# Bebra777228/PolGen-RVC

Measured on AMD Instinct MI355X. Metric: real-time-factor (audio-sec/wall-sec) per GPU, 30s@16kHz RMVPE->48kHz, higher is better.
Workload: dtype f32 (conv products as 3 fp16 MFMAs of a hi/lo split, fp32 accumulate; fp32 elsewhere)

## Files before the change

### include/rvcx.h

```cpp
#ifndef RVCX_H
#define RVCX_H
#include <stdint.h>

#ifdef __cplusplus
extern "C" {
#endif

typedef struct rvcx_ctx rvcx_ctx;

typedef struct {
  const char* name;
  const void* data;
  int32_t dtype;
  int32_t ndim;
  int64_t shape[4];
} rvcx_tensor;

typedef struct {
  int32_t inter_channels, hidden_channels, filter_channels, n_heads, n_layers, kernel_size;
  int32_t n_resblocks;
  int32_t res_kernels[4];
  int32_t res_dilations[4][3];
  int32_t n_ups;
  int32_t up_rates[6], up_kernels[6];
// ... 175 lines not shown
  float reverb_rm_size, reverb_wet, reverb_dry, reverb_damping, reverb_width;
  float low_shelf_gain, high_shelf_gain;
  float compressor_ratio, compressor_threshold;
  float noise_gate_threshold, noise_gate_ratio, noise_gate_attack, noise_gate_release;
  float chorus_rate_hz, chorus_depth, chorus_centre_delay_ms, chorus_feedback, chorus_mix;
  int32_t sample_rate, channels;
} rvcx_fx_params;
int rvcx_fx_chain(rvcx_ctx*, int B, const float* const* x_hd, const int64_t* n, const rvcx_fx_params*, float* const* y_hd);
int rvcx_op_fx_highpass(rvcx_ctx*, const float* x_hd, int64_t n, int channels, int sr, float fc, float* y_hd);
int rvcx_op_fx_compressor(rvcx_ctx*, const float* x_hd, int64_t n, int channels, int sr, float ratio, float threshold_db,
                          float attack_ms, float release_ms, float* y_hd, float* env_hd);
int rvcx_op_fx_gate(rvcx_ctx*, const float* x_hd, int64_t n, int channels, int sr, float threshold_db, float ratio,
                    float attack_ms, float release_ms, float* y_hd, float* env_hd);
int rvcx_op_fx_reverb(rvcx_ctx*, const float* x_hd, int64_t n, int channels, int sr, float room_size, float damping, float wet,
                      float dry, float width, float* y_hd);
int rvcx_op_fx_shelf(rvcx_ctx*, const float* x_hd, int64_t n, int channels, int sr, int high, float gain_db, float fc, float Q,
                     float* y_hd);
int rvcx_op_fx_chorus(rvcx_ctx*, const float* x_hd, int64_t n, int channels, int sr, float rate_hz, float depth,
                      float centre_delay_ms, float feedback, float mix, float* y_hd);
int rvcx_op_fx_mix(rvcx_ctx*, const int16_t* vocal_hd, int64_t n_v, const int16_t* inst_hd, int64_t n_i, float vocal_gain_db,
                   float inst_gain_db, int16_t* out_hd);
int rvcx_fx_chunk(void);
int rvcx_fx_last_passes(rvcx_ctx*, int32_t* passes3);
float rvcx_fx_cte(double ms, int sr);
int rvcx_fx_delay(int sr, int D);
int rvcx_fx_coeffs(int kind, int sr, double fc, double Q, double gain_db, float* coef5);
int rvcx_fx_highpass_host(const float* x, int64_t n, int sr, float fc, float* y);
int rvcx_fx_biquad_host(const float* x, int64_t n, const float* coef5, float* y);
int rvcx_fx_follower_host(const float* x, int64_t n, int square, int sqrt_out, float c_attack, float c_release, float* env);
int rvcx_fx_compressor_host(const float* x, int64_t n, int sr, float ratio, float threshold_db, float attack_ms,
                            float release_ms, float* y, float* env);
int rvcx_fx_gate_host(const float* x, int64_t n, int sr, float threshold_db, float ratio, float attack_ms, float release_ms,
                      float* y, float* env);
int rvcx_fx_comb_host(const float* in, int64_t n, int D, float fb, float d, float* out);
int rvcx_fx_allpass_host(const float* in, int64_t n, int D, float* out);
int rvcx_fx_chorus_host(const float* x, int64_t n, int sr, float rate_hz, float depth, float centre_delay_ms, float feedback,
                        float mix, float* y);
int rvcx_fx_mix_host(const int16_t* vocal, int64_t n_v, const int16_t* inst, int64_t n_i, float vocal_gain_db,
                     float inst_gain_db, int16_t* out);

int rvcx_stream_open_fx(rvcx_ctx*, int model_id, const rvcx_stream_cfg*, const rvcx_stream_io*, const rvcx_fx_params* fx,
                        const rvcx_params* p, const int32_t* sid, const float* pitch, int* stream_id);
int rvcx_stream_out_channels(rvcx_ctx*, int stream_id);
int rvcx_stream_set_fx(rvcx_ctx*, int stream_id, const rvcx_fx_params*);
int rvcx_stream_last_fx_ms(rvcx_ctx*, int stream_id, float* ms8);
int rvcx_op_stream_fx(rvcx_ctx*, const float* x_hd, int S, int64_t frames, int channels, int sr, int block_frames,
                      const rvcx_fx_params* fx, uint32_t stage_mask, float* y_hd);
int rvcx_fx_reverb_host(const float* x, int64_t n, int sr, float room_size, float damping, float wet, float dry, float width,
                        float* y);

int rvcx_last_timing(rvcx_ctx*, float* ms9);
int rvcx_conv_profile(rvcx_ctx*, int begin, int64_t* launches, double* flops, double* ms, int32_t* bm,
                      int32_t* bn, int32_t* kind, int cap);
const char* rvcx_conv_profile_csv(rvcx_ctx*);
int rvcx_device_info(int device, char* name, int name_cap, int64_t* total_bytes);
int rvcx_mem_info(rvcx_ctx*, int64_t* free_bytes, int64_t* total_bytes);
int64_t rvcx_fp32_reruns(rvcx_ctx*);
int64_t rvcx_fp32_layers(rvcx_ctx*);
int rvcx_fp32_pinned(rvcx_ctx*, char* buf, int cap);
int64_t rvcx_gru_fallbacks(rvcx_ctx*);
int rvcx_gru_publish_probe(rvcx_ctx*);
int64_t rvcx_index_exhaustive(rvcx_ctx*);

int rvcx_kmeans(rvcx_ctx*, const float* x_hd, int64_t n, int dim, const float* init_hd, int k, int iters,
                float* centroids_hd, int32_t* assign_hd, int32_t* counts_hd, double* objective, int32_t* splits);
int rvcx_ivf_assign(rvcx_ctx*, const float* x_hd, int64_t n, int dim, const float* centroids_hd, int nlist,
                    int32_t* assign_hd);
int rvcx_index_features(rvcx_ctx*, int B, const float* wav_hd, int64_t n, int out_dim, float* feats_hd);
int64_t rvcx_kmeans_exhaustive(rvcx_ctx*);

int rvcx_debug_inject(rvcx_ctx*, int what);
double rvcx_flop_counter(rvcx_ctx*, int reset);
void* rvcx_stream(rvcx_ctx*);

int rvcx_op_fcpe_post(rvcx_ctx*, const float* raw_hd, int F_in, int p_len, double pitch, double f0_min, double f0_max,
                      int32_t* coarse, float* f0);
int rvcx_op_conv1d(rvcx_ctx*, const float* x, const float* w, const float* bias, const float* res,
                   float* y, int B, int Cin, int Tin, int Cout, int K, int stride, int dil,
                   int pad_left, int Tout, int groups, int pre_lrelu, float pre_slope, int act,
                   float act_slope, const int32_t* lens_in, const int32_t* lens_out);
int rvcx_op_resblock_pair(rvcx_ctx*, const float* x, const float* w1, const float* b1, const float* w2,
                          const float* b2, float* y, int B, int C, int T, int K, int dil, float slope, int fused,
                          const int32_t* lens);
int rvcx_op_resblock3(rvcx_ctx*, const float* x, const float* w1, const float* b1, const float* w2, const float* b2,
                      float* y, int B, int C, int T, const int32_t* dils, float slope, const int32_t* lens);
int rvcx_bench_resblock_pair(rvcx_ctx*, int B, int C, int T, int K, int dil, int fused, int iters,
                             float* ms_per_launch);
int rvcx_bench_conv1d(rvcx_ctx*, int B, int Cin, int Tin, int Cout, int K, int stride, int dil, int groups,
                      int iters, float* ms_per_launch);
int rvcx_conv_override(int tile, int variant, int splitk);
int rvcx_op_convtranspose1d(rvcx_ctx*, const float* x, const float* w, const float* bias, float* y,
                            int B, int Cin, int Tin, int Cout, int K, int stride, int pad,
                            int pre_lrelu, float pre_slope);
int rvcx_op_conv2d3x3(rvcx_ctx*, const float* x, const float* w, const float* bias, const float* res,
                      float* y, int B, int Cin, int H, int W, int Cout, int act);
int rvcx_op_convblock2d(rvcx_ctx*, const float* x, const float* w1, const float* b1, const float* w2, const float* b2,
                        const float* wsc, const float* bsc, float* y, int B, int Cin, int Cout, int H, int W,
                        const int32_t* rows);
int rvcx_op_convtranspose2d(rvcx_ctx*, const float* x, const float* w, const float* bias, float* y,
                            int B, int Cin, int H, int W, int Cout, int act);
int rvcx_op_attention(rvcx_ctx*, const float* q, const float* k, const float* v, float* out, int B,
                      int H, int D, int T, float scale, const float* emb_rel_k,
                      const float* emb_rel_v, int window, const int32_t* lens);
int rvcx_op_gemm_tm(rvcx_ctx*, const float* x_cf, const float* w, const float* bias, const float* res_tm, int B, int T,
                    int Cin, int Cout, int act, int exact_fp32, float* y_tm, float* y_cf, float* y_split);
int rvcx_bench_gemm(rvcx_ctx*, int64_t rows, int Cin, int Cout, int iters, float* ms_per_launch);
int rvcx_op_layernorm_tm(rvcx_ctx*, const float* x, const float* gamma, const float* beta, float* y, float* y_split,
                         int64_t rows, int C, float eps);
int rvcx_op_layernorm_c(rvcx_ctx*, const float* x, const float* gamma, const float* beta, float* y,
                        int B, int C, int T, float eps);
int rvcx_op_groupnorm_gelu(rvcx_ctx*, const float* x, const float* gamma, const float* beta, int B, int C, int T, float eps,
                           const int32_t* lens, float* y, float* stats, float* y_split);
int rvcx_op_hubert_conv0(rvcx_ctx*, const float* wav, const float* w, const float* gamma, const float* beta, int B, int C,
                         int n, int K, int stride, float eps, const int32_t* lens, int fused, float* stats, float* y_split,
                         uint16_t* raw_split);
int rvcx_op_sine_source(rvcx_ctx*, const float* f0, const float* noise, const float* lin_wb, int B, int T, int upp, float sr,
                        const int32_t* lens, float* har);
int rvcx_op_randn(rvcx_ctx*, int64_t n, uint64_t seed, uint64_t offset, float* out);
int rvcx_op_reflect_pad(rvcx_ctx*, const float* x, int B, int n, int p, const int32_t* ns, float* y);
int rvcx_op_mel_post(rvcx_ctx*, const float* mel, int B, int nmel, int F, int Tp, const float* bn, const int32_t* fs,
                     const int32_t* tps, float* out);
int rvcx_op_decode_f0(rvcx_ctx*, const float* sal, int B, int T, int ld, float thred, float f0_min, float f0_max, float* f0);
int rvcx_op_avgpool2(rvcx_ctx*, const float* x, int planes, int H, int Wp, int64_t x_ps, int64_t y_ps, float* y);
int rvcx_op_gru_input(rvcx_ctx*, const float* x, int B, int C, int T, int Wp, float* y);
int rvcx_op_upsample_protect(rvcx_ctx*, const float* feats, const float* feats0, const float* pitchf, int C, int Th, int p_len,
                             float protect, int use_protect, int ld_in, int ld_out, float* out);
int rvcx_op_bigru(rvcx_ctx*, const float* x, const float* w_ih, const float* w_hh, const float* b_ih,
                  const float* b_hh, const float* w_ih_r, const float* w_hh_r, const float* b_ih_r,
                  const float* b_hh_r, float* y, int B, int T, int I, int H);
int rvcx_op_highpass(rvcx_ctx*, const double* x, double* y, int64_t n);
int rvcx_highpass_exact(const double* x, double* y, int64_t n);

int64_t rvcx_flac_encode_bound(int64_t frames, int channels);
int64_t rvcx_flac_encode_s16(const int16_t* pcm, int64_t frames, int channels, int sample_rate, uint8_t* out, int64_t cap);
int rvcx_flac_info(const uint8_t* data, int64_t n, int64_t* frames, int32_t* channels, int32_t* sample_rate, int32_t* bits);
int64_t rvcx_flac_decode_s32(const uint8_t* data, int64_t n, int32_t* out, int64_t cap_samples);
const char* rvcx_flac_last_error(void);

#ifdef __cplusplus
}
#endif
#endif
```

### polgen-rvc_amd/_lib.py

```python
from __future__ import annotations

import ctypes as C
import os
import threading
import types
from typing import Optional, Sequence

import numpy as np

_HERE = os.path.dirname(os.path.abspath(__file__))
LIB_PATH = os.environ.get("RVCX_LIBRARY") or os.path.join(_HERE, "librvcx.so")


class RvcxError(RuntimeError):
    pass


class Tensor(C.Structure):
    _fields_ = [("name", C.c_char_p), ("data", C.c_void_p), ("dtype", C.c_int32),
                ("ndim", C.c_int32), ("shape", C.c_int64 * 4)]


class SynthCfg(C.Structure):
    _fields_ = [("inter_channels", C.c_int32), ("hidden_channels", C.c_int32),
# ... 49 lines not shown
class FxParams(C.Structure):
    _fields_ = [(k, C.c_float) for k in FX_FIELDS] + [("sample_rate", C.c_int32), ("channels", C.c_int32)]

    @classmethod
    def make(cls, values, sample_rate, channels=2):
        p = cls()
        if isinstance(values, dict):
            values = [values[k] for k in FX_FIELDS]
        if len(values) != len(FX_FIELDS):
            raise RvcxError(f"FxParams: {len(FX_FIELDS)} effect values expected, got {len(values)}")
        for k, v in zip(FX_FIELDS, values):
            setattr(p, k, float(v))
        p.sample_rate, p.channels = int(sample_rate), int(channels)
        return p


FX_UI_DEFAULTS = dict(reverb_rm_size=0.1, reverb_wet=0.1, reverb_dry=0.8, reverb_damping=0.9, reverb_width=1.0,
                      low_shelf_gain=0, high_shelf_gain=0, compressor_ratio=4, compressor_threshold=-12,
                      noise_gate_threshold=-40, noise_gate_ratio=8, noise_gate_attack=10, noise_gate_release=100,
                      chorus_rate_hz=0, chorus_depth=0, chorus_centre_delay_ms=0, chorus_feedback=0, chorus_mix=0)


class StreamIO(C.Structure):
    _fields_ = [("in_rate", C.c_int32), ("in_channels", C.c_int32), ("out_rate", C.c_int32), ("reserved", C.c_int32)]


def stream_resample_delay(sr_in: int, sr_out: int) -> int:
    return int(lib().rvcx_stream_resample_delay(int(sr_in), int(sr_out)))


class StreamCfg(C.Structure):
    _fields_ = [("n_streams", C.c_int32), ("block_frames", C.c_int32), ("context_frames", C.c_int32),
                ("crossfade_frames", C.c_int32), ("search_frames", C.c_int32)]


def head_from_rate(T: int, rate) -> int:
    return int(int(T) * (1.0 - float(np.float32(rate))))


def sola_reference(y, b, Lb, Lx, Ls, offset=None):
    y, b = np.asarray(y, np.float64), np.asarray(b, np.float64)
    Lb, Lx, Ls = int(Lb), int(Lx), int(Ls)
    assert y.shape == (Lb + Lx + Ls,) and b.shape == (Lx,)
    win = np.lib.stride_tricks.sliding_window_view(y[:Ls + Lx], Lx)
    den = np.sqrt((win * win).sum(1) + 1e-8)
    scores = (win @ b) / den
    mags = (np.abs(win) @ np.abs(b)) / den
    d = int(np.argmax(scores)) if offset is None else int(offset)
    out = y[d:d + Lb].copy()
    k = min(Lx, Lb)
    fin = np.sin(0.5 * np.pi * np.arange(Lx) / max(Lx - 1, 1)) ** 2
    out[:k] = y[d:d + k] * fin[:k] + b[:k] * (1.0 - fin[:k])
    return out, y[d + Lb:d + Lb + Lx].copy(), d, scores, mags


_lib = None

SYMBOLS = [
    "rvcx_create", "rvcx_destroy", "rvcx_last_error", "rvcx_version", "rvcx_load_hubert",
    "rvcx_load_rmvpe", "rvcx_index_exhaustive", "rvcx_load_crepe", "rvcx_crepe_frames", "rvcx_crepe_predict", "rvcx_op_crepe_decode", "rvcx_get_f0_crepe_x", "rvcx_load_fcpe", "rvcx_fcpe_f0", "rvcx_fcpe_frames", "rvcx_get_f0_fcpe_x", "rvcx_op_fcpe_post", "rvcx_load_synth", "rvcx_unload_synth", "rvcx_load_index", "rvcx_load_index_ivf",
    "rvcx_weights_regions", "rvcx_weights_adopt", "rvcx_weights_clone", "rvcx_rmvpe_f0", "rvcx_rmvpe_frames", "rvcx_rmvpe_mel", "rvcx_synth_infer_taps", "rvcx_hubert_features",
    "rvcx_hubert_frames", "rvcx_synth_infer", "rvcx_synth_infer_window", "rvcx_synth_dec_rf", "rvcx_synth_upp", "rvcx_index_blend",
    "rvcx_out_len", "rvcx_convert_batch", "rvcx_convert_batch_f64", "rvcx_micro_batch", "rvcx_bucket_length", "rvcx_last_micro_batches", "rvcx_last_cuts", "rvcx_noise_len",
    "rvcx_get_f0", "rvcx_get_f0_x", "rvcx_vc", "rvcx_vc_frames", "rvcx_last_timing",
    "rvcx_flop_counter", "rvcx_fp32_reruns", "rvcx_mem_info", "rvcx_conv_profile", "rvcx_conv_profile_csv", "rvcx_stream", "rvcx_op_conv1d", "rvcx_op_resblock_pair", "rvcx_bench_resblock_pair", "rvcx_bench_conv1d", "rvcx_conv_override", "rvcx_op_convtranspose1d",
    "rvcx_op_conv2d3x3", "rvcx_op_convblock2d", "rvcx_op_convtranspose2d", "rvcx_op_attention", "rvcx_op_layernorm_c",
    "rvcx_op_bigru", "rvcx_op_highpass", "rvcx_highpass_exact", "rvcx_convert_batch_ex", "rvcx_get_f0_x_ex", "rvcx_fp32_layers", "rvcx_fp32_pinned",
    "rvcx_gru_fallbacks", "rvcx_gru_publish_probe", "rvcx_debug_inject", "rvcx_f0_file_track", "rvcx_op_gemm_tm", "rvcx_op_layernorm_tm",
    "rvcx_resample_len", "rvcx_resample_f64", "rvcx_resample_f64_kind", "rvcx_bench_gemm", "rvcx_device_info",
    "rvcx_convert_submit", "rvcx_convert_wait", "rvcx_convert_poll", "rvcx_convert_inflight", "rvcx_ticket_lead_ms",
    "rvcx_synth_infer_head", "rvcx_op_sola", "rvcx_stream_open", "rvcx_stream_step", "rvcx_stream_reset", "rvcx_stream_close",
    "rvcx_stream_out_len", "rvcx_stream_noise_len", "rvcx_stream_frames",
    "rvcx_stream_open_io", "rvcx_stream_in_len", "rvcx_stream_delays", "rvcx_stream_resample_delay", "rvcx_stream_last_taps",
    "rvcx_stream_set", "rvcx_op_stream_resample",
    "rvcx_stream_open_fx", "rvcx_stream_out_channels", "rvcx_stream_set_fx", "rvcx_stream_last_fx_ms", "rvcx_op_stream_fx",
    "rvcx_fx_reverb_host",
    "rvcx_fx_chain", "rvcx_op_fx_highpass", "rvcx_op_fx_compressor", "rvcx_op_fx_gate", "rvcx_op_fx_reverb", "rvcx_op_fx_shelf",
    "rvcx_op_fx_chorus", "rvcx_op_fx_mix", "rvcx_fx_chunk", "rvcx_fx_last_passes", "rvcx_fx_cte", "rvcx_fx_delay",
    "rvcx_fx_coeffs", "rvcx_fx_highpass_host", "rvcx_fx_biquad_host", "rvcx_fx_follower_host", "rvcx_fx_compressor_host",
    "rvcx_fx_gate_host", "rvcx_fx_comb_host", "rvcx_fx_allpass_host", "rvcx_fx_chorus_host", "rvcx_fx_mix_host",
    "rvcx_op_groupnorm_gelu", "rvcx_op_hubert_conv0", "rvcx_op_sine_source", "rvcx_op_randn", "rvcx_op_reflect_pad",
    "rvcx_op_mel_post", "rvcx_op_decode_f0", "rvcx_op_avgpool2", "rvcx_op_gru_input", "rvcx_op_upsample_protect",
    "rvcx_kmeans", "rvcx_ivf_assign", "rvcx_kmeans_exhaustive", "rvcx_index_features",
    "rvcx_op_resblock3", "rvcx_flac_encode_bound", "rvcx_flac_encode_s16", "rvcx_flac_info", "rvcx_flac_decode_s32", "rvcx_flac_last_error",
]


def lib() -> C.CDLL:
    global _lib
    if _lib is None:
        if not os.path.exists(LIB_PATH):
            raise RvcxError(f"{LIB_PATH} not built (run `make` / __graft_entry__.build()); "
                            "rvcx has no CPU fallback")
        _lib = C.CDLL(LIB_PATH)
        _lib.rvcx_last_error.restype = C.c_char_p
        _lib.rvcx_version.restype = C.c_char_p
        _lib.rvcx_flop_counter.restype = C.c_double
        _lib.rvcx_stream.restype = C.c_void_p
        _lib.rvcx_conv_profile_csv.restype = C.c_char_p
        _lib.rvcx_out_len.restype = C.c_int64
        _lib.rvcx_fp32_reruns.restype = C.c_int64
        _lib.rvcx_fp32_layers.restype = C.c_int64
        _lib.rvcx_gru_fallbacks.restype = C.c_int64
        _lib.rvcx_bucket_length.restype = C.c_int64
        _lib.rvcx_last_cuts.restype = C.c_int64
        _lib.rvcx_last_cuts.argtypes = [C.c_void_p, C.c_void_p, C.c_int64]
        _lib.rvcx_resample_len.restype = C.c_int64
        _lib.rvcx_noise_len.restype = C.c_int64
        _lib.rvcx_crepe_frames.restype = C.c_int64
        _lib.rvcx_index_exhaustive.restype = C.c_int64
        _lib.rvcx_kmeans_exhaustive.restype = C.c_int64
        _lib.rvcx_kmeans.argtypes = [C.c_void_p, C.c_void_p, C.c_int64, C.c_int, C.c_void_p, C.c_int, C.c_int, C.c_void_p,
                                     C.c_void_p, C.c_void_p, C.c_void_p, C.c_void_p]
        _lib.rvcx_ivf_assign.argtypes = [C.c_void_p, C.c_void_p, C.c_int64, C.c_int, C.c_void_p, C.c_int, C.c_void_p]
        _lib.rvcx_flac_encode_bound.restype = C.c_int64
        _lib.rvcx_flac_encode_s16.restype = C.c_int64
        _lib.rvcx_flac_decode_s32.restype = C.c_int64
        _lib.rvcx_flac_last_error.restype = C.c_char_p
        _lib.rvcx_flac_encode_bound.argtypes = [C.c_int64, C.c_int]
        _lib.rvcx_flac_encode_s16.argtypes = [C.c_void_p, C.c_int64, C.c_int, C.c_int, C.c_void_p, C.c_int64]
        _lib.rvcx_flac_info.argtypes = [C.c_void_p, C.c_int64, C.POINTER(C.c_int64), C.POINTER(C.c_int32),
                                        C.POINTER(C.c_int32), C.POINTER(C.c_int32)]
        _lib.rvcx_flac_decode_s32.argtypes = [C.c_void_p, C.c_int64, C.c_void_p, C.c_int64]
        _lib.rvcx_convert_submit.argtypes = [C.c_void_p, C.c_int, C.c_int, C.c_void_p, C.c_int, C.c_void_p, C.c_void_p,
                                             C.c_void_p, C.c_void_p, C.c_void_p, C.c_void_p, C.c_void_p,
                                             C.POINTER(C.c_int64)]
        _lib.rvcx_convert_wait.argtypes = [C.c_void_p, C.c_int64]
        _lib.rvcx_convert_poll.argtypes = [C.c_void_p, C.c_int64]
        _lib.rvcx_convert_inflight.argtypes = [C.c_void_p]
        _lib.rvcx_ticket_lead_ms.argtypes = [C.c_void_p, C.c_int64]
        _lib.rvcx_ticket_lead_ms.restype = C.c_float
        _lib.rvcx_stream_out_len.restype = C.c_int64
        _lib.rvcx_stream_noise_len.restype = C.c_int64
        _lib.rvcx_stream_out_len.argtypes = [C.c_void_p, C.c_int]
        _lib.rvcx_stream_noise_len.argtypes = [C.c_void_p, C.c_int]
        _lib.rvcx_stream_frames.argtypes = [C.c_void_p, C.c_int]
        _lib.rvcx_stream_in_len.restype = C.c_int64
        _lib.rvcx_stream_in_len.argtypes = [C.c_void_p, C.c_int]
        _lib.rvcx_stream_resample_delay.argtypes = [C.c_int, C.c_int]
        _lib.rvcx_stream_set.argtypes = [C.c_void_p, C.c_int, C.c_void_p, C.c_void_p, C.c_float, C.c_float]
        _lib.rvcx_op_stream_resample.argtypes = [C.c_void_p, C.c_void_p, C.c_int, C.c_int64, C.c_int, C.c_int, C.c_int, C.c_int,
                                                 C.c_void_p]
        fp, ip, vp = C.POINTER(C.c_float), C.POINTER(C.c_int32), C.c_void_p
        _lib.rvcx_op_groupnorm_gelu.argtypes = [vp, fp, fp, fp, C.c_int, C.c_int, C.c_int, C.c_float, ip, fp, fp, fp]
        _lib.rvcx_op_hubert_conv0.argtypes = [vp, fp, fp, fp, fp, C.c_int, C.c_int, C.c_int, C.c_int, C.c_int, C.c_float, ip,
                                              C.c_int, fp, fp, C.POINTER(C.c_uint16)]
        _lib.rvcx_op_sine_source.argtypes = [vp, fp, fp, fp, C.c_int, C.c_int, C.c_int, C.c_float, ip, fp]
        _lib.rvcx_op_randn.argtypes = [vp, C.c_int64, C.c_uint64, C.c_uint64, fp]
        _lib.rvcx_op_reflect_pad.argtypes = [vp, fp, C.c_int, C.c_int, C.c_int, ip, fp]
        _lib.rvcx_op_mel_post.argtypes = [vp, fp, C.c_int, C.c_int, C.c_int, C.c_int, fp, ip, ip, fp]
        _lib.rvcx_op_decode_f0.argtypes = [vp, fp, C.c_int, C.c_int, C.c_int, C.c_float, C.c_float, C.c_float, fp]
        _lib.rvcx_op_avgpool2.argtypes = [vp, fp, C.c_int, C.c_int, C.c_int, C.c_int64, C.c_int64, fp]
        _lib.rvcx_op_gru_input.argtypes = [vp, fp, C.c_int, C.c_int, C.c_int, C.c_int, fp]
        _lib.rvcx_op_upsample_protect.argtypes = [vp, fp, fp, fp, C.c_int, C.c_int, C.c_int, C.c_float, C.c_int, C.c_int,
                                                  C.c_int, fp]
        f, d, i, i64 = C.c_float, C.c_double, C.c_int, C.c_int64
        _lib.rvcx_fx_chain.argtypes = [vp, i, vp, vp, C.POINTER(FxParams), vp]
        _lib.rvcx_op_fx_highpass.argtypes = [vp, vp, i64, i, i, f, vp]
        _lib.rvcx_op_fx_compressor.argtypes = [vp, vp, i64, i, i, f, f, f, f, vp, vp]
        _lib.rvcx_op_fx_gate.argtypes = [vp, vp, i64, i, i, f, f, f, f, vp, vp]
        _lib.rvcx_op_fx_reverb.argtypes = [vp, vp, i64, i, i, f, f, f, f, f, vp]
        _lib.rvcx_op_fx_shelf.argtypes = [vp, vp, i64, i, i, i, f, f, f, vp]
        _lib.rvcx_op_fx_chorus.argtypes = [vp, vp, i64, i, i, f, f, f, f, f, vp]
        _lib.rvcx_op_fx_mix.argtypes = [vp, vp, i64, vp, i64, f, f, vp]
        _lib.rvcx_fx_last_passes.argtypes = [vp, vp]
        _lib.rvcx_fx_cte.argtypes, _lib.rvcx_fx_cte.restype = [d, i], f
# ... 369 lines not shown
        self.effects = values

    def last_fx_ms(self):
        ms = (C.c_float * 8)()
        self._ctx._ck(lib().rvcx_stream_last_fx_ms(self._ctx._h, self.id, ms), "stream_last_fx_ms")
        names = ["highpass", "compressor", "gate", "reverb", "low_shelf", "high_shelf", "chorus", "total"]
        return dict(zip(names, [float(v) for v in ms]))

    def reset(self):
        self._ctx._ck(lib().rvcx_stream_reset(self._ctx._h, self.id), "stream_reset")

    def close(self):
        if self.id is not None and getattr(self._ctx, "_h", None):
            sid, self.id = self.id, None
            self._ctx._ck(lib().rvcx_stream_close(self._ctx._h, sid), "stream_close")
        self.id = None

    def __enter__(self):
        return self

    def __exit__(self, *exc):
        self.close()
        return False


class Context:

    regions_on_device = True

    def __init__(self, device: int = 0):
        self._h = C.c_void_p()
        rc = lib().rvcx_create(int(device), C.byref(self._h))
        if rc != 0:
            raise RvcxError("rvcx_create: " + (lib().rvcx_last_error(None) or b"").decode())
        self.device = device
        self.lock = threading.RLock()

    def close(self):
        if getattr(self, "_h", None):
            lib().rvcx_destroy(self._h)
            self._h = None

    def __del__(self):
        try:
            self.close()
        except Exception:
            pass

    def _ck(self, rc, what):
        if rc != 0:
            raise RvcxError(f"{what}: " + (lib().rvcx_last_error(self._h) or b"").decode())

    def conv1d(self, x, w, bias=None, res=None, stride=1, dil=1, pad_left=0, Tout=None, groups=1,
               pre_lrelu=None, act=0, act_slope=0.0, lens_in=None, lens_out=None):
        x, w = f32(x), f32(w)
        B, Cin, Tin = x.shape
        Cout, _, K = w.shape
        if Tout is None:
            Tout = (Tin + 2 * pad_left - dil * (K - 1) - 1) // stride + 1
        y = np.empty((B, Cout, Tout), np.float32)
        bias = None if bias is None else f32(bias)
        res = None if res is None else f32(res)
        li, lo = i32(lens_in), i32(lens_out)
        self._ck(lib().rvcx_op_conv1d(self._h, _p(x), _p(w), _p(bias), _p(res), _p(y), B, Cin, Tin, Cout, K,
                                      stride, dil, pad_left, Tout, groups,
                                      0 if pre_lrelu is None else 1,
                                      C.c_float(0.0 if pre_lrelu is None else pre_lrelu), act,
                                      C.c_float(act_slope), _p(li, C.c_int32), _p(lo, C.c_int32)), "op_conv1d")
        return y

    def resblock_pair(self, x, w1, b1, w2, b2, dil=1, slope=0.1, fused=True, lens=None):
        x, w1, w2 = f32(x), f32(w1), f32(w2)
        B, Cc, T = x.shape
        K = w1.shape[2]
        y = np.empty_like(x)
        b1 = None if b1 is None else f32(b1)
        b2 = None if b2 is None else f32(b2)
        li = i32(lens)
        self._ck(lib().rvcx_op_resblock_pair(self._h, _p(x), _p(w1), _p(b1), _p(w2), _p(b2), _p(y), B, Cc, T, K, dil,
                                             C.c_float(slope), 1 if fused else 0, _p(li, C.c_int32)),
                 "op_resblock_pair")
        return y

    def resblock3(self, x, w1, b1, w2, b2, dils=(1, 3, 5), slope=0.1, lens=None):
        x, w1, w2 = f32(x), f32(w1), f32(w2)
        B, Cc, T = x.shape
        y = np.empty_like(x)
        b1 = None if b1 is None else f32(b1)
        b2 = None if b2 is None else f32(b2)
        d = i32(list(dils))
        li = i32(lens)
        self._ck(lib().rvcx_op_resblock3(self._h, _p(x), _p(w1), _p(b1), _p(w2), _p(b2), _p(y), B, Cc, T, _p(d, C.c_int32),
                                         C.c_float(slope), _p(li, C.c_int32)), "op_resblock3")
        return y

    def bench_resblock_pair(self, B, Cc, T, K, dil=1, fused=True, iters=10):
        ms = C.c_float(0)
        self._ck(lib().rvcx_bench_resblock_pair(self._h, B, Cc, T, K, dil, 1 if fused else 0, iters, C.byref(ms)),
                 "bench_resblock_pair")
        return ms.value, 4.0 * B * Cc * Cc * K * T / (ms.value * 1e-3) / 1e12

    @staticmethod
    def conv_override(tile=-1, variant=-1, splitk=-1):
        if lib().rvcx_conv_override(tile, variant, splitk) != 0:
            raise RvcxError("conv_override: " + (lib().rvcx_last_error(None) or b"").decode())

    def bench_conv1d(self, B, Cin, Tin, Cout, K, stride=1, dil=1, groups=1, iters=10):
        ms = C.c_float(0)
        self._ck(lib().rvcx_bench_conv1d(self._h, B, Cin, Tin, Cout, K, stride, dil, groups, iters, C.byref(ms)),
                 "bench_conv1d")
        pad = (K * dil - dil) // 2
        Tout = (Tin + 2 * pad - dil * (K - 1) - 1) // stride + 1
        flops = 2.0 * B * Cout * Tout * K * (Cin // groups)
        return ms.value, flops / (ms.value * 1e-3) / 1e12

    def convtranspose1d(self, x, w, bias=None, stride=1, pad=0, pre_lrelu=None):
        x, w = f32(x), f32(w)
        B, Cin, Tin = x.shape
        _, Cout, K = w.shape
        Tout = (Tin - 1) * stride - 2 * pad + K
        y = np.empty((B, Cout, Tout), np.float32)
        bias = None if bias is None else f32(bias)
        self._ck(lib().rvcx_op_convtranspose1d(self._h, _p(x), _p(w), _p(bias), _p(y), B, Cin, Tin, Cout, K,
                                               stride, pad, 0 if pre_lrelu is None else 1,
                                               C.c_float(0.0 if pre_lrelu is None else pre_lrelu)),
                 "op_convtranspose1d")
        return y

    def conv2d3x3(self, x, w, bias=None, res=None, act=0):
        x, w = f32(x), f32(w)
        B, Cin, H, W = x.shape
        Cout = w.shape[0]
        y = np.empty((B, Cout, H, W), np.float32)
        bias = None if bias is None else f32(bias)
        res = None if res is None else f32(res)
        self._ck(lib().rvcx_op_conv2d3x3(self._h, _p(x), _p(w), _p(bias), _p(res), _p(y), B, Cin, H, W, Cout,
                                         act), "op_conv2d3x3")
        return y

    def convblock2d(self, x, w1, b1, w2, b2, wsc=None, bsc=None, rows=None):
        x, w1, w2 = f32(x), f32(w1), f32(w2)
        B, Cin, H, W = x.shape
        Cout = w1.shape[0]
        y = np.empty((B, Cout, H, W), np.float32)
        b1 = None if b1 is None else f32(b1)
        b2 = None if b2 is None else f32(b2)
        wsc = None if wsc is None else f32(wsc)
        bsc = None if bsc is None else f32(bsc)
        ri = i32(rows)
        self._ck(lib().rvcx_op_convblock2d(self._h, _p(x), _p(w1), _p(b1), _p(w2), _p(b2), _p(wsc), _p(bsc), _p(y), B, Cin,
                                           Cout, H, W, _p(ri, C.c_int32)), "op_convblock2d")
        return y

    def convtranspose2d(self, x, w, bias=None, act=0):
        x, w = f32(x), f32(w)
        B, Cin, H, W = x.shape
        Cout = w.shape[1]
        y = np.empty((B, Cout, 2 * H, 2 * W), np.float32)
        bias = None if bias is None else f32(bias)
        self._ck(lib().rvcx_op_convtranspose2d(self._h, _p(x), _p(w), _p(bias), _p(y), B, Cin, H, W, Cout, act),
                 "op_convtranspose2d")
        return y

    def attention(self, q, k, v, heads, scale, emb_rel_k=None, emb_rel_v=None, window=10, lens=None):
        q, k, v = f32(q), f32(k), f32(v)
        B, HD, T = q.shape
# ... 825 lines not shown
```

### polgen-rvc_amd/csrc/api_ops.hip

```cpp
#include "api_internal.h"
#include "h3_device.h"

using namespace rvcx;
using namespace rvcx::api;

static void to_host(Ctx& c, float* h, const float* d, size_t n) {
  RVCX_HIP(hipMemcpyAsync(h, d, n * sizeof(float), hipMemcpyDeviceToHost, c.stream));
  RVCX_HIP(hipStreamSynchronize(c.stream));
}
#define TEMP_REGION(C) WeightRegion tmp_region_; RegionScope tmp_scope_(*(C), tmp_region_)

extern "C" {

int rvcx_op_conv1d(rvcx_ctx* ctx, const float* x, const float* w, const float* bias, const float* res,
                   float* y, int B, int Cin, int Tin, int Cout, int K, int stride, int dil,
                   int pad_left, int Tout, int groups, int pre_lrelu, float pre_slope, int act,
                   float act_slope, const int32_t* lens_in, const int32_t* lens_out) {
  API_BEGIN(ctx)
  TEMP_REGION(C);
  size_t nx = (size_t)B * Cin * Tin, ny = (size_t)B * Cout * Tout;
  C->arena.reserve((nx + 2 * ny) * 4 + (64 << 20));
  C->arena.reset();
  ConvW L = make_conv(*C, w, bias, Cout, Cin / groups, K, groups, true);
  float* dx = to_dev(*C, x, nx);
// ... 12 lines not shown
  to_host(*C, y, dy, ny);
  C->arena.reset();
  API_END
}

int rvcx_op_resblock_pair(rvcx_ctx* ctx, const float* x, const float* w1, const float* b1, const float* w2,
                          const float* b2, float* y, int B, int Cc, int T, int K, int dil, float slope, int fused,
                          const int32_t* lens) {
  API_BEGIN(ctx)
  TEMP_REGION(C);
  const size_t n = (size_t)B * Cc * T;
  C->arena.reserve(n * 4 * 4 + (64 << 20));
  C->arena.reset();
  ConvW L1 = make_conv(*C, w1, b1, Cc, Cc, K, 1, true);
  ConvW L2 = make_conv(*C, w2, b2, Cc, Cc, K, 1, true);
  float* dx = to_dev(*C, x, n);
  float* dt = C->arena.alloc<float>(n);
  float* dy = C->arena.alloc<float>(n);
  RVCX_HIP(hipMemsetAsync(dy, 0xff, n * 4, C->stream));
  const int* dl = (lens ? to_dev(*C, lens, B) : nullptr);
  if (fused) {
    PairArgs pa;
    pa.x = dx;
    pa.y = dy;
    pa.w1 = (L1.w_h3 && *L1.h3_ok) ? L1.w_h3 : nullptr;
    pa.w2 = (L2.w_h3 && *L2.h3_ok) ? L2.w_h3 : nullptr;
    pa.b1 = L1.bias;
    pa.b2 = L2.bias;
    pa.lens = dl;
    pa.B = B;
    pa.C = Cc;
    pa.T = T;
    pa.bs = (long)Cc * T;
    pa.cs = T;
    pa.k = K;
    pa.dil = dil;
    pa.slope = slope;
    if (!resblock_pair_ok(pa) && !g_force_fp32) fail("resblock pair: shape not supported by the fused kernel");
  }
  if (fused && !g_force_fp32) {
    PairArgs pa;
    pa.x = dx;
    pa.y = dy;
    pa.w1 = L1.w_h3;
    pa.w2 = L2.w_h3;
    pa.b1 = L1.bias;
    pa.b2 = L2.bias;
    pa.lens = dl;
    pa.B = B;
    pa.C = Cc;
    pa.T = T;
    pa.bs = (long)Cc * T;
    pa.cs = T;
    pa.k = K;
    pa.dil = dil;
    pa.slope = slope;
    C->pair_on(pa, C->stream);
  } else {
    ConvArgs a = conv1d_args(L1, dx, dt, B, T, T, 1, dil, (K * dil - dil) / 2);
    a.pre_act = ACT_LRELU;
    a.pre_slope = slope;
    a.act = ACT_LRELU;
    a.act_slope = slope;
    a.lens_in = dl;
    a.lens_out = dl;
    ConvArgs a2 = conv1d_args(L2, dt, dy, B, T, T, 1, 1, (K - 1) / 2);
    const bool split = conv_h3_split_ok(a) && conv_h3_split_ok(a2);
    if (split) {
      a.y_split = dt;
      a.y = nullptr;
    }
    C->conv(a);
    if (split) a2.x_split = dt;
    conv_set_res(a2, dx, Cc, T);
    a2.lens_in = dl;
    a2.lens_out = dl;
    C->conv(a2);
  }
  to_host(*C, y, dy, n);
  C->arena.reset();
  API_END
}

int rvcx_op_resblock3(rvcx_ctx* ctx, const float* x, const float* w1, const float* b1, const float* w2, const float* b2,
                      float* y, int B, int Cc, int T, const int32_t* dils, float slope, const int32_t* lens) {
  API_BEGIN(ctx)
  TEMP_REGION(C);
  const size_t n = (size_t)B * Cc * T, wn = (size_t)Cc * Cc * 3;
  C->arena.reserve(n * 4 * 3 + (64 << 20));
  C->arena.reset();
  ConvW L1[3], L2[3];
  for (int s = 0; s < 3; ++s) {
    L1[s] = make_conv(*C, w1 + s * wn, b1 ? b1 + (size_t)s * Cc : nullptr, Cc, Cc, 3, 1, true);
    L2[s] = make_conv(*C, w2 + s * wn, b2 ? b2 + (size_t)s * Cc : nullptr, Cc, Cc, 3, 1, true);
  }
  float* dx = to_dev(*C, x, n);
  float* dy = C->arena.alloc<float>(n);
  RVCX_HIP(hipMemsetAsync(dy, 0xff, n * 4, C->stream));
  const int* dl = (lens ? to_dev(*C, lens, B) : nullptr);
  Block3Args a;
  a.x = dx;
  a.y = dy;
  for (int s = 0; s < 3; ++s) {
    a.w1[s] = (L1[s].w_h3 && *L1[s].h3_ok) ? L1[s].w_h3 : nullptr;
    a.w2[s] = (L2[s].w_h3 && *L2[s].h3_ok) ? L2[s].w_h3 : nullptr;
    a.b1[s] = L1[s].bias;
    a.b2[s] = L2[s].bias;
    a.dil[s] = dils ? dils[s] : 2 * s + 1;
  }
  a.ovf_layer = L1[0].ovf_word;
  a.lens = dl;
  a.B = B;
  a.C = Cc;
  a.T = T;
  a.bs = (long)Cc * T;
  a.cs = T;
  a.slope = slope;
  a.any_shape = true;
  if (!resblock3_ok(a)) fail("resblock3: shape not supported by the whole-block kernel");
  C->block3_on(a, C->stream);
  to_host(*C, y, dy, n);
  C->arena.reset();
  API_END
}

int rvcx_bench_resblock_pair(rvcx_ctx* ctx, int B, int Cc, int T, int K, int dil, int fused, int iters,
                             float* ms_per_launch) {
  REQUIRE_DEBUG(ctx, "rvcx_bench_resblock_pair")
  API_BEGIN(ctx)
  TEMP_REGION(C);
  const size_t n = (size_t)B * Cc * T;
  C->arena.reserve(n * 4 * 4 + (64 << 20));
  C->arena.reset();
  std::vector<float> w((size_t)Cc * Cc * K), bias((size_t)Cc, 0.1f);
  for (size_t i = 0; i < w.size(); ++i) w[i] = ((float)((i * 2654435761u) % 2001) / 1000.f - 1.f) / std::sqrt((float)Cc * K);
  ConvW L1 = make_conv(*C, w.data(), bias.data(), Cc, Cc, K, 1, true);
  ConvW L2 = make_conv(*C, w.data(), bias.data(), Cc, Cc, K, 1, true);
  float* dx = C->arena.alloc<float>(n);
  float* dt = C->arena.alloc<float>(n);
  float* dy = C->arena.alloc<float>(n);
  launch_randn(dx, n, 1, 0, C->stream);
  if (getenv("RVCX_BENCH_ZERO")) RVCX_HIP(hipMemsetAsync(dx, 0, n * 4, C->stream));
  PairArgs pa;
  pa.x = dx;
  pa.y = dy;
  pa.w1 = L1.w_h3;
  pa.w2 = L2.w_h3;
  pa.b1 = L1.bias;
  pa.b2 = L2.bias;
  pa.B = B;
  pa.C = Cc;
  pa.T = T;
  pa.bs = (long)Cc * T;
  pa.cs = T;
  pa.k = K;
  pa.dil = dil;
  ConvArgs a = conv1d_args(L1, dx, dt, B, T, T, 1, dil, (K * dil - dil) / 2);
  a.pre_act = ACT_LRELU;
  a.pre_slope = 0.1f;
  a.act = ACT_LRELU;
  a.act_slope = 0.1f;
  ConvArgs a2 = conv1d_args(L2, dt, dy, B, T, T, 1, 1, (K - 1) / 2);
  const bool split = conv_h3_split_ok(a) && conv_h3_split_ok(a2);
  if (split) {
    a.y_split = dt;
    a.y = nullptr;
    a2.x_split = dt;
  }
  conv_set_res(a2, dx, Cc, T);
  auto once = [&]() {
    if (fused) {
      C->pair_on(pa, C->stream);
    } else {
      C->conv(a);
      C->conv(a2);
    }
  };
  if (fused && !resblock_pair_ok(pa)) fail("resblock pair: shape not supported by the fused kernel");
  once();
  if (fused && getenv("RVCX_PAIR_TRACE")) {
    const size_t cap = (size_t)B * (T / 32 + 64) * 8;
    long long* tr = C->arena.alloc<long long>(cap);
    RVCX_HIP(hipMemsetAsync(tr, 0, cap * 8, C->stream));
    pa.trace = tr;
    once();
    pa.trace = nullptr;
    std::vector<long long> h(cap);
    RVCX_HIP(hipMemcpyAsync(h.data(), tr, cap * 8, hipMemcpyDeviceToHost, C->stream));
    RVCX_HIP(hipStreamSynchronize(C->stream));
    if (FILE* f = fopen(getenv("RVCX_PAIR_TRACE"), "a")) {
      fprintf(f, "# C %d T %d K %d dil %d\n", Cc, T, K, dil);
      for (size_t w = 0; w * 8 < cap; ++w)
        if (h[w * 8]) {
          for (int k = 0; k < 8; ++k) fprintf(f, "%lld%c", h[w * 8 + k], k == 7 ? '\n' : ',');
        }
      fclose(f);
    }
  }
  hipEvent_t e0, e1;
  RVCX_HIP(hipEventCreate(&e0));
  RVCX_HIP(hipEventCreate(&e1));
  RVCX_HIP(hipEventRecord(e0, C->stream));
  for (int i = 0; i < iters; ++i) once();
  RVCX_HIP(hipEventRecord(e1, C->stream));
  RVCX_HIP(hipEventSynchronize(e1));
  float ms = 0.f;
  RVCX_HIP(hipEventElapsedTime(&ms, e0, e1));
  *ms_per_launch = ms / iters;
  (void)hipEventDestroy(e0);
  (void)hipEventDestroy(e1);
  C->arena.reset();
  API_END
}

int rvcx_conv_override(int tile, int variant, int splitk) {
  REQUIRE_DEBUG(nullptr, "rvcx_conv_override")
  rvcx::g_conv_override.tile = tile;
  rvcx::g_conv_override.variant = variant;
  rvcx::g_conv_override.splitk = splitk;
  return 0;
}

int rvcx_bench_conv1d(rvcx_ctx* ctx, int B, int Cin, int Tin, int Cout, int K, int stride, int dil, int groups,
                      int iters, float* ms_per_launch) {
  REQUIRE_DEBUG(ctx, "rvcx_bench_conv1d")
  API_BEGIN(ctx)
  TEMP_REGION(C);
  const int pad = (K * dil - dil) / 2;
  const int Tout = (Tin + 2 * pad - dil * (K - 1) - 1) / stride + 1;
  size_t nx = (size_t)B * Cin * Tin, ny = (size_t)B * Cout * Tout;
  C->arena.reserve((nx + 2 * ny) * 4 + (64 << 20));
  C->arena.reset();
  std::vector<float> w((size_t)Cout * (Cin / groups) * K), bias((size_t)Cout, 0.1f);
  for (size_t i = 0; i < w.size(); ++i) w[i] = (float)((i * 2654435761u) % 2001) / 1000.f - 1.f;
  ConvW L = make_conv(*C, w.data(), bias.data(), Cout, Cin / groups, K, groups, true);
  float* dx = C->arena.alloc<float>(nx);
  float* dy = C->arena.alloc<float>(ny);
  float* dr = C->arena.alloc<float>(ny);
  launch_randn(dx, nx, 1, 0, C->stream);
  launch_randn(dr, ny, 2, 0, C->stream);
  ConvArgs a = conv1d_args(L, dx, dy, B, Tin, Tout, stride, dil, pad);
  conv_set_res(a, dr, Cout, Tout);
  a.pre_act = ACT_LRELU;
  a.pre_slope = 0.1f;
  C->conv(a);
  long long* dtrace = nullptr;
  const long ntrace = 1L << 16;
  if (getenv("RVCX_TRACE")) {
    RVCX_HIP(hipMalloc(&dtrace, ntrace * 6 * sizeof(long long)));
    RVCX_HIP(hipMemset(dtrace, 0, ntrace * 6 * sizeof(long long)));
    a.trace = dtrace;
  }
  hipEvent_t e0, e1;
  RVCX_HIP(hipEventCreate(&e0));
  RVCX_HIP(hipEventCreate(&e1));
  RVCX_HIP(hipEventRecord(e0, C->stream));
  for (int i = 0; i < iters; ++i) C->conv(a);
  RVCX_HIP(hipEventRecord(e1, C->stream));
  RVCX_HIP(hipEventSynchronize(e1));
  float ms = 0.f;
  RVCX_HIP(hipEventElapsedTime(&ms, e0, e1));
  *ms_per_launch = ms / iters;
  if (dtrace) {
    std::vector<long long> ht((size_t)ntrace * 6);
    RVCX_HIP(hipMemcpy(ht.data(), dtrace, ht.size() * sizeof(long long), hipMemcpyDeviceToHost));
    FILE* f = fopen(getenv("RVCX_TRACE"), "w");
    for (long i = 0; i < ntrace; ++i)
      if (ht[i * 6 + 5]) fprintf(f, "%ld,%lld,%lld,%lld,%lld,%lld,%lld\n", i, ht[i*6], ht[i*6+1], ht[i*6+2], ht[i*6+3], ht[i*6+4], ht[i*6+5]);
    fclose(f);
    (void)hipFree(dtrace);
  }
  (void)hipEventDestroy(e0);
  (void)hipEventDestroy(e1);
  C->arena.reset();
  API_END
}

int rvcx_op_convtranspose1d(rvcx_ctx* ctx, const float* x, const float* w, const float* bias, float* y,
                            int B, int Cin, int Tin, int Cout, int K, int stride, int pad,
                            int pre_lrelu, float pre_slope) {
  API_BEGIN(ctx)
  TEMP_REGION(C);
  const int Tout = (Tin - 1) * stride - 2 * pad + K;
  size_t nx = (size_t)B * Cin * Tin, ny = (size_t)B * Cout * Tout;
  C->arena.reserve((nx + ny) * 4 + (64 << 20));
  C->arena.reset();
  ConvT1dW L = make_convT1d(*C, w, bias, Cin, Cout, K, stride, pad);
  float* dx = to_dev(*C, x, nx);
  float* dy = C->arena.alloc<float>(ny);
  ConvArgs a = convT1d_args(L, dx, dy, B, Tin, Tout);
  if (pre_lrelu) {
    a.pre_act = ACT_LRELU;
    a.pre_slope = pre_slope;
  }
  C->conv(a);
  to_host(*C, y, dy, ny);
  C->arena.reset();
  API_END
}

static std::vector<float> pad_rows(const float* x, size_t planes, int H, int W) {
  const int Wp = W + 2;
  std::vector<float> o(planes * H * Wp, 0.f);
  for (size_t p = 0; p < planes; ++p)
    for (int h = 0; h < H; ++h)
// ... 584 lines not shown
```

### polgen-rvc_amd/csrc/attention.hip

```cpp
#include <cstdlib>

#include "conv.h"
#include "conv_device.h"
#include "ops.h"

namespace rvcx {

constexpr int KT = 32;
constexpr int VROW = 33;

template <int DT>
__global__ __launch_bounds__(256) void attn_kernel(const float* __restrict__ q, const float* __restrict__ k,
                                                   const float* __restrict__ v, float* __restrict__ out,
                                                   float* __restrict__ m_out, float* __restrict__ l_out,
                                                   const float* __restrict__ relq, int H, int D, int T,
                                                   int ld, long in_bs, long out_bs, float scale, int window,
                                                   const int* lens, int nsplit, float* opart) {
  __shared__ float Ks[32 * DT * KT];
  __shared__ float Vs[32 * DT * VROW];
  const int tid = threadIdx.x, lane = tid & 63, wave = tid >> 6;
  const int i = lane & 31, h = lane >> 5;
  const int b = blockIdx.z, hd = blockIdx.y;
  const int qblk = blockIdx.x / nsplit, split = blockIdx.x - qblk * nsplit;
  const int q0 = qblk * 128 + wave * 32;
  const int len = lens ? lens[b] : T;
  const long base = (long)b * in_bs + (long)hd * D * ld;
  const long obase = (long)b * out_bs + (long)hd * D * ld;
  const float* qb = q + base;
  const float* kb = k + base;
  const float* vb = v + base;
  const int nsteps = D / 2;

  float qreg[16 * DT];
  const int qi = q0 + i;
#pragma unroll
  for (int s = 0; s < 16 * DT; ++s) {
    float val = 0.f;
    if (s < nsteps && qi < T) val = qb[(long)(2 * s + h) * ld + qi] * scale;
    qreg[s] = val;
  }

  f32x16 acc_o[DT];
#pragma unroll
  for (int dt = 0; dt < DT; ++dt)
#pragma unroll
    for (int r = 0; r < 16; ++r) acc_o[dt][r] = 0.f;
  float m_run = -INFINITY, l_run = 0.f;
  const int nrel = 2 * window + 1;
  const float* relrow = relq ? relq + (((long)b * H + hd) * T + min(qi, T - 1)) * nrel : nullptr;

  const int tiles = (len + KT - 1) / KT;
  const int klo = (int)((long)tiles * split / nsplit) * KT;
  const int khi = min(len, (int)((long)tiles * (split + 1) / nsplit) * KT);
  for (int k0 = klo; k0 < khi; k0 += KT) {
    __syncthreads();
    for (int idx = tid; idx < 32 * DT * KT; idx += 256) {
      const int d = idx / KT, kk = idx % KT;
      const int key = k0 + kk;
      float kv = 0.f, vv = 0.f;
      if (d < D && key < len) {
        kv = kb[(long)d * ld + key];
        vv = vb[(long)d * ld + key];
      }
      Ks[d * KT + kk] = kv;
      Vs[d * VROW + kk] = vv;
    }
    __syncthreads();
    f32x16 sacc;
#pragma unroll
    for (int r = 0; r < 16; ++r) sacc[r] = 0.f;
#pragma unroll
    for (int s = 0; s < 16 * DT; ++s) {
      if (s < nsteps) {
        const float a = Ks[(2 * s + h) * KT + i];
        sacc = __builtin_amdgcn_mfma_f32_32x32x2f32(a, qreg[s], sacc, 0, 0, 0);
      }
    }
    const bool band = relq && (k0 <= q0 + 31 + window) && (k0 + KT - 1 >= q0 - window);
    float mloc = -INFINITY;
#pragma unroll
    for (int r = 0; r < 16; ++r) {
      const int key = k0 + (r & 3) + 8 * (r >> 2) + 4 * h;
      float sv = sacc[r];
      if (band) {
        const int rel = key - qi + window;
        if (rel >= 0 && rel < nrel && qi < T) sv += relrow[rel];
      }
      if (key >= len) sv = -INFINITY;
      sacc[r] = sv;
// ... 16 lines not shown
#pragma unroll
      for (int r = 0; r < 16; ++r) acc_o[dt][r] *= alpha;
#pragma unroll
    for (int s = 0; s < 16; ++s) {
      const int kidx = (s & 3) + 8 * (s >> 2) + 4 * h;
#pragma unroll
      for (int dt = 0; dt < DT; ++dt) {
        const float a = Vs[(dt * 32 + i) * VROW + kidx];
        acc_o[dt] = __builtin_amdgcn_mfma_f32_32x32x2f32(a, sacc[s], acc_o[dt], 0, 0, 0);
      }
    }
  }
  if (nsplit > 1) {
    if (qi < T) {
      const int DP = 32 * DT;
      float* pb = opart + (((long)b * H + hd) * nsplit + split) * (DP + 2) * T;
#pragma unroll
      for (int dt = 0; dt < DT; ++dt)
#pragma unroll
        for (int r = 0; r < 16; ++r) {
          const int d = dt * 32 + (r & 3) + 8 * (r >> 2) + 4 * h;
          pb[(long)d * T + qi] = acc_o[dt][r];
        }
      if (h == 0) {
        pb[(long)DP * T + qi] = m_run;
        pb[(long)(DP + 1) * T + qi] = l_run;
      }
    }
    return;
  }
  if (qi < T) {
    const float inv = 1.f / l_run;
    float* ob = out + obase;
#pragma unroll
    for (int dt = 0; dt < DT; ++dt)
#pragma unroll
      for (int r = 0; r < 16; ++r) {
        const int d = dt * 32 + (r & 3) + 8 * (r >> 2) + 4 * h;
        if (d < D) ob[(long)d * ld + qi] = (qi < len) ? acc_o[dt][r] * inv : 0.f;
      }
    if (m_out && h == 0) {
      m_out[((long)b * H + hd) * T + qi] = m_run;
      l_out[((long)b * H + hd) * T + qi] = l_run;
    }
  }
}

typedef _Float16 ahalf8 __attribute__((ext_vector_type(8)));
constexpr float kAttS = 256.f;
#ifndef RVCX_ATT_ABL
#define RVCX_ATT_ABL 0
#endif
constexpr int kAttAbl = RVCX_ATT_ABL;
__device__ __forceinline__ f32x16 att_mfma(ahalf8 a, ahalf8 b, f32x16 c) {
#if defined(__HIP_DEVICE_COMPILE__)
  return __builtin_amdgcn_mfma_f32_32x32x16_f16(a, b, c, 0, 0, 0);
#else
  return c;
#endif
}

struct AttRsrc {
#if defined(__HIP_DEVICE_COMPILE__)
  __amdgpu_buffer_rsrc_t r;
#endif
};
__device__ __forceinline__ AttRsrc att_rsrc(const float* base, int bytes) {
  AttRsrc b;
#if defined(__HIP_DEVICE_COMPILE__)
  b.r = __builtin_amdgcn_make_buffer_rsrc(const_cast<float*>(base), 0, bytes, 0x00020000);
#endif
  return b;
}
__device__ __forceinline__ float att_load(const AttRsrc& b, int off) {
#if defined(__HIP_DEVICE_COMPILE__)
  return __builtin_bit_cast(float, __builtin_amdgcn_raw_buffer_load_b32(b.r, off, 0, 0));
#else
  return 0.f;
#endif
}
constexpr int kAttOob = 0x7ffffff0;

template <int DT>
__global__ __launch_bounds__(256) void att_presplit_kernel(const float* __restrict__ k, const float* __restrict__ v,
                                                           uint4* __restrict__ kimg, uint4* __restrict__ vimg, int H, int D,
                                                           int T, int ld, long in_bs, const int* lens, int* ovf_word,
                                                           int* ovf_layer, int seq) {
  constexpr int NS = 2 * DT;
  constexpr int K_ELEMS = NS * 2 * 32, V_ELEMS = DT * 2 * 2 * 32;
  const int kt = blockIdx.x, hd = blockIdx.y, b = blockIdx.z, tid = threadIdx.x;
  const int len = lens ? lens[b] : T;
  const int k0 = kt * 32;
  const long base = (long)b * in_bs + (long)hd * D * ld;
  const float* kb = k + base;
  const float* vb = v + base;
  uint4* ko = kimg + (((long)b * H + hd) * gridDim.x + kt) * (2 * K_ELEMS);
  uint4* vo = vimg + (((long)b * H + hd) * gridDim.x + kt) * (2 * V_ELEMS);
  bool ovf = false;
  for (int e0 = tid; e0 < K_ELEMS; e0 += 256) {
    const int key = e0 & 31, hh = (e0 >> 5) & 1, s = e0 >> 6;
    ahalf8 a0, a2;
#pragma unroll
    for (int e = 0; e < 8; ++e) {
      const int d = 16 * s + 8 * hh + e;
      const float val = (d < D && k0 + key < len) ? kb[(long)d * ld + k0 + key] : 0.f;
      ovf |= !(fabsf(val) < kH3ActLimit / kAttS);
      const _Float16 vh = (_Float16)val;
      a0[e] = (_Float16)((float)vh * kAttS);
      a2[e] = (_Float16)((val - (float)vh) * kAttS);
    }
    ko[((s * 2 + 0) * 2 + hh) * 32 + key] = __builtin_bit_cast(uint4, a0);
    ko[((s * 2 + 1) * 2 + hh) * 32 + key] = __builtin_bit_cast(uint4, a2);
  }
  for (int e0 = tid; e0 < V_ELEMS; e0 += 256) {
    const int dd = e0 & 31, hh = (e0 >> 5) & 1, s2 = (e0 >> 6) & 1, dt = e0 >> 7;
    const int d = dt * 32 + dd;
    ahalf8 a0, a2;
#pragma unroll
    for (int e = 0; e < 8; ++e) {
      const int r = 8 * s2 + e;
      const int key = k0 + (r & 3) + 8 * (r >> 2) + 4 * hh;
      const float val = (d < D && key < len) ? vb[(long)d * ld + key] : 0.f;
      ovf |= !(fabsf(val) < kH3ActLimit / kAttS);
      const _Float16 vh = (_Float16)val;
      a0[e] = (_Float16)((float)vh * kAttS);
      a2[e] = (_Float16)((val - (float)vh) * kAttS);
    }
    vo[(((dt * 2 + s2) * 2 + 0) * 2 + hh) * 32 + dd] = __builtin_bit_cast(uint4, a0);
    vo[(((dt * 2 + s2) * 2 + 1) * 2 + hh) * 32 + dd] = __builtin_bit_cast(uint4, a2);
  }
  if (ovf) report_h3_overflow(ovf_word, ovf_layer, seq);
}

typedef unsigned att_u32x4 __attribute__((ext_vector_type(4)));
template <int NKE, int NVE>
__device__ __forceinline__ void att_fetch(att_u32x4 (&rk)[NKE], att_u32x4 (&rv)[NVE], const uint4* __restrict__ kp,
                                          const uint4* __restrict__ vp, int tid) {
#pragma unroll
  for (int j = 0; j < NKE; ++j) rk[j] = *reinterpret_cast<const att_u32x4*>(kp + tid + 256 * j);
#pragma unroll
  for (int j = 0; j < NVE; ++j) rv[j] = *reinterpret_cast<const att_u32x4*>(vp + tid + 256 * j);
}
template <int NKE, int NVE>
__device__ __forceinline__ void att_commit(const att_u32x4 (&rk)[NKE], const att_u32x4 (&rv)[NVE], uint4* Ks, uint4* Vs,
                                           int tid) {
#pragma unroll
  for (int j = 0; j < NKE; ++j) *reinterpret_cast<att_u32x4*>(Ks + tid + 256 * j) = rk[j];
#pragma unroll
  for (int j = 0; j < NVE; ++j) *reinterpret_cast<att_u32x4*>(Vs + tid + 256 * j) = rv[j];
}

template <int DT>
__global__ __launch_bounds__(256, 2) void attn_h3_kernel(const float* __restrict__ q, const uint4* __restrict__ kimg,
                                                      const uint4* __restrict__ vimg, float* __restrict__ out,
                                                      float* __restrict__ m_out, float* __restrict__ l_out,
                                                      const float* __restrict__ relq, int H, int D, int T,
                                                      int ld, long in_bs, long out_bs, float scale, int window,
                                                      const int* lens, int nsplit, float* opart, int* ovf_word,
                                                      int* ovf_layer, int seq) {
  constexpr int NS = 2 * DT;
  __shared__ uint4 Ks[NS * 2 * 2 * 32];
  __shared__ uint4 Vs[DT * 2 * 2 * 2 * 32];
  const int tid = threadIdx.x, lane = tid & 63, wave = tid >> 6;
  const int i = lane & 31, h = lane >> 5;
  const int b = blockIdx.z, hd = blockIdx.y;
  const int qblk = blockIdx.x / nsplit, split = blockIdx.x - qblk * nsplit;
  const int q0 = qblk * 128 + wave * 32;
  const int len = lens ? lens[b] : T;
  const long base = (long)b * in_bs + (long)hd * D * ld;
  const long obase = (long)b * out_bs + (long)hd * D * ld;
  const float* qb = q + base;

  bool ovf = false;
  ahalf8 qh[NS], ql[NS];
  const int qi = q0 + i;
#pragma unroll
  for (int s = 0; s < NS; ++s)
#pragma unroll
    for (int e = 0; e < 8; ++e) {
      const int d = 16 * s + 8 * h + e;
      const float val = (d < D && qi < T) ? qb[(long)d * ld + qi] * scale : 0.f;
      ovf |= !(fabsf(val) < kH3ActLimit);
      const _Float16 vh = (_Float16)val;
      qh[s][e] = vh;
      ql[s][e] = (_Float16)((val - (float)vh) * kAttS);
    }

  f32x16 acc_o[DT];
#pragma unroll
  for (int dt = 0; dt < DT; ++dt)
#pragma unroll
    for (int r = 0; r < 16; ++r) acc_o[dt][r] = 0.f;
  float m_run = -INFINITY, l_run = 0.f;
  const int nrel = 2 * window + 1;
  const float* relrow = relq ? relq + (((long)b * H + hd) * T + min(qi, T - 1)) * nrel : nullptr;

  constexpr float invS = 1.f / kAttS;
  constexpr int KSZ = NS * 2 * 2 * 32, VSZ = DT * 2 * 2 * 2 * 32;
  constexpr int NKE = KSZ / 256, NVE = VSZ / 256;
  static_assert(KSZ % 256 == 0 && VSZ % 256 == 0, "image sizes are multiples of the workgroup");
  const int ntile = (T + 31) / 32;
  const uint4* kt_base = kimg + ((long)b * H + hd) * ntile * KSZ;
  const uint4* vt_base = vimg + ((long)b * H + hd) * ntile * VSZ;
  att_u32x4 rk[NKE], rv[NVE];
  auto fetch = [&](int k0) {
    att_fetch<NKE, NVE>(rk, rv, kt_base + (long)(k0 >> 5) * KSZ, vt_base + (long)(k0 >> 5) * VSZ, tid);
  };
  auto commit = [&]() { att_commit<NKE, NVE>(rk, rv, Ks, Vs, tid); };

  const int tiles = (len + 31) / 32;
  const int klo = (int)((long)tiles * split / nsplit) * 32;
  const int khi = min(len, (int)((long)tiles * (split + 1) / nsplit) * 32);
  if (klo < khi) fetch(klo);
  for (int k0 = klo; k0 < khi; k0 += 32) {
// ... 76 lines not shown
        acc_o[dt] = att_mfma(a0, ph[s2], acc_o[dt]);
        acc_o[dt] = att_mfma(a1, pl[s2], acc_o[dt]);
        acc_o[dt] = att_mfma(a2, ph[s2], acc_o[dt]);
      }
  }
  if (ovf) report_h3_overflow(ovf_word, ovf_layer, seq);
#pragma unroll
  for (int dt = 0; dt < DT; ++dt)
#pragma unroll
    for (int r = 0; r < 16; ++r) acc_o[dt][r] *= invS;
  if (nsplit > 1) {
    if (qi < T) {
      const int DP = 32 * DT;
      float* pb = opart + (((long)b * H + hd) * nsplit + split) * (DP + 2) * T;
#pragma unroll
      for (int dt = 0; dt < DT; ++dt)
#pragma unroll
        for (int r = 0; r < 16; ++r) {
          const int d = dt * 32 + (r & 3) + 8 * (r >> 2) + 4 * h;
          pb[(long)d * T + qi] = acc_o[dt][r];
        }
      if (h == 0) {
        pb[(long)DP * T + qi] = m_run;
        pb[(long)(DP + 1) * T + qi] = l_run;
      }
    }
    return;
  }
  if (qi < T) {
    const float inv = 1.f / l_run;
    float* ob = out + obase;
#pragma unroll
    for (int dt = 0; dt < DT; ++dt)
#pragma unroll
      for (int r = 0; r < 16; ++r) {
        const int d = dt * 32 + (r & 3) + 8 * (r >> 2) + 4 * h;
        if (d < D) ob[(long)d * ld + qi] = (qi < len) ? acc_o[dt][r] * inv : 0.f;
      }
    if (m_out && h == 0) {
      m_out[((long)b * H + hd) * T + qi] = m_run;
      l_out[((long)b * H + hd) * T + qi] = l_run;
    }
  }
}


__global__ __launch_bounds__(256) void attn_merge_kernel(const float* __restrict__ opart, float* __restrict__ out,
                                                         float* m_out, float* l_out, int H, int D, int DP, int T, int ld,
                                                         long out_bs, int nsplit, const int* lens) {
  const int t = blockIdx.x * 64 + (threadIdx.x & 63), part = threadIdx.x >> 6;
  const int hd = blockIdx.y >> 2, dq = blockIdx.y & 3, b = blockIdx.z;
  if (t >= T) return;
  const float* pb = opart + (((long)b * H + hd) * nsplit) * (DP + 2) * T;
  const long ss = (long)(DP + 2) * T;
  float ms[8], w[8];
  float m = -INFINITY, l = 0.f;
#pragma unroll
  for (int s = 0; s < 8; ++s) {
    ms[s] = s < nsplit ? pb[s * ss + (long)DP * T + t] : -INFINITY;
    m = fmaxf(m, ms[s]);
  }
#pragma unroll
  for (int s = 0; s < 8; ++s) {
    w[s] = (ms[s] == -INFINITY) ? 0.f : expf(ms[s] - m);
    if (s < nsplit) l += w[s] * pb[s * ss + (long)(DP + 1) * T + t];
  }
  const int len = lens ? lens[b] : T;
  const float inv = 1.f / l;
  float* ob = out + (long)b * out_bs + (long)hd * D * ld;
  const int dper = (D + 3) / 4, d0 = dq * dper, d1 = min(D, d0 + dper);
  for (int d = d0 + part; d < d1; d += 4) {
    float acc = 0.f;
#pragma unroll
    for (int s = 0; s < 8; ++s)
      if (s < nsplit) acc += w[s] * pb[s * ss + (long)d * T + t];
    ob[(long)d * ld + t] = t < len ? acc * inv : 0.f;
  }
  if (m_out && part == 0 && dq == 0) {
    m_out[((long)b * H + hd) * T + t] = m;
    l_out[((long)b * H + hd) * T + t] = l;
  }
}

__global__ __launch_bounds__(256) void rel_logits_kernel(const float* __restrict__ q, const float* __restrict__ ek,
                                                         float* __restrict__ relq, int H, int D, int T, int ld,
                                                         long in_bs, float scale, int nrel) {
  extern __shared__ float eks[];
  for (int idx = threadIdx.x; idx < nrel * D; idx += 256) eks[idx] = ek[idx];
  __syncthreads();
  const int tq = threadIdx.x & 63, part = __builtin_amdgcn_readfirstlane(threadIdx.x >> 6);
  const int nmine = part < nrel ? (nrel - part + 3) / 4 : 0;
  const int t = blockIdx.x * 64 + tq;
  const int hd = blockIdx.y, b = blockIdx.z;
  if (t >= T) return;
  const float* qb = q + (long)b * in_bs + (long)hd * D * ld;
  float acc[8];
#pragma unroll
  for (int i = 0; i < 8; ++i) acc[i] = 0.f;
  int d = 0;
  for (; d + 8 <= D; d += 8) {
    float qv[8];
#pragma unroll
    for (int u = 0; u < 8; ++u) qv[u] = qb[(long)(d + u) * ld + t] * scale;
#pragma unroll
    for (int i = 0; i < 8; ++i)
      if (i < nmine) {
        const float* e = eks + (part + 4 * i) * D + d;
        if ((D & 3) == 0) {
          const float4 e0 = *reinterpret_cast<const float4*>(e), e1 = *reinterpret_cast<const float4*>(e + 4);
          acc[i] = fmaf(qv[0], e0.x, acc[i]);
          acc[i] = fmaf(qv[1], e0.y, acc[i]);
          acc[i] = fmaf(qv[2], e0.z, acc[i]);
          acc[i] = fmaf(qv[3], e0.w, acc[i]);
          acc[i] = fmaf(qv[4], e1.x, acc[i]);
          acc[i] = fmaf(qv[5], e1.y, acc[i]);
          acc[i] = fmaf(qv[6], e1.z, acc[i]);
          acc[i] = fmaf(qv[7], e1.w, acc[i]);
        } else {
#pragma unroll
          for (int u = 0; u < 8; ++u) acc[i] = fmaf(qv[u], e[u], acc[i]);
        }
      }
  }
  for (; d < D; ++d) {
    const float qv = qb[(long)d * ld + t] * scale;
#pragma unroll
    for (int i = 0; i < 8; ++i)
      if (i < nmine) acc[i] = fmaf(qv, eks[(part + 4 * i) * D + d], acc[i]);
  }
  float* o = relq + (((long)b * H + hd) * T + t) * nrel;
#pragma unroll
  for (int i = 0; i < 8; ++i) {
    const int r = part + 4 * i;
    if (r < nrel) o[r] = acc[i];
  }
}

__global__ __launch_bounds__(256) void rel_values_kernel(const float* __restrict__ q, const float* __restrict__ k,
                                                         const float* __restrict__ relq,
                                                         const float* __restrict__ m_in,
                                                         const float* __restrict__ l_in,
                                                         const float* __restrict__ ev, float* __restrict__ out,
                                                         int H, int D, int T, int ld, long in_bs, long out_bs, float scale,
                                                         int window, const int* lens) {
  extern __shared__ float sm[];
  const int nrel = 2 * window + 1;
  const int KW = 32 + 2 * window;
  float* evs = sm;
  float* ps = evs + nrel * D;
  float* qs = ps + 32 * (nrel + 1);
  float* ks = qs + D * 32;
  const int tq = threadIdx.x & 31, part = threadIdx.x >> 5;
  const int hd = blockIdx.y, b = blockIdx.z;
  const int tb = blockIdx.x * 32;
  const int t = tb + tq;
  const int len = lens ? lens[b] : T;
  const long base = (long)b * in_bs + (long)hd * D * ld;
  const long obase = (long)b * out_bs + (long)hd * D * ld;
  for (int idx = threadIdx.x; idx < nrel * D; idx += 256) evs[idx] = ev[idx];
  for (int idx = threadIdx.x; idx < D * 32; idx += 256) {
    const int d = idx >> 5, j = idx & 31;
    qs[idx] = tb + j < T ? q[base + (long)d * ld + tb + j] * scale : 0.f;
  }
  for (int idx = threadIdx.x; idx < D * KW; idx += 256) {
    const int d = idx / KW, j = idx - d * KW;
    const int key = tb - window + j;
    ks[idx] = (key >= 0 && key < T) ? k[base + (long)d * ld + key] : 0.f;
  }
  __syncthreads();
  if (t < T) {
    const float m = m_in[((long)b * H + hd) * T + t], l = l_in[((long)b * H + hd) * T + t];
    for (int r = part; r < nrel; r += 8) {
      const int key = t + r - window;
      float p = 0.f;
      if (key >= 0 && key < len) {
        float s = 0.f;
        for (int d = 0; d < D; ++d) s = fmaf(qs[d * 32 + tq], ks[d * KW + tq + r], s);
        s += relq[(((long)b * H + hd) * T + t) * nrel + r];
        p = expf(s - m) / l;
      }
      ps[tq * (nrel + 1) + r] = p;
    }
  }
  __syncthreads();
  if (t < T && t < len) {
    for (int d = part; d < D; d += 8) {
      float acc = 0.f;
      for (int r = 0; r < nrel; ++r) acc = fmaf(ps[tq * (nrel + 1) + r], evs[r * D + d], acc);
      out[obase + (long)d * ld + t] += acc;
    }
  }
}

void launch_attention(const float* q, const float* k, const float* v, float* out, int B, int H, int D, int T,
                      int ld, long in_bs, long out_bs, float scale, const float* emb_rel_k, const float* emb_rel_v, int window,
                      const int* lens, float* scratch, float* split_scratch, hipStream_t stream, int* ovf, int* ovf_layer,
                      int seq, bool allow_h3) {
  RVCX_CHECK(D % 2 == 0 && D <= 96, "attention: head dim must be even and <= 96");
  const int nrel = 2 * window + 1;
  float *relq = nullptr, *mb = nullptr, *lb = nullptr;
  if (emb_rel_k) {
    RVCX_CHECK(nrel <= 32 && scratch != nullptr, "attention: window too large / no scratch");
    relq = scratch;
    mb = relq + (size_t)B * H * T * nrel;
    lb = mb + (size_t)B * H * T;
    hipLaunchKernelGGL(rel_logits_kernel, dim3(cdiv(T, 64), H, B), dim3(256), nrel * D * sizeof(float), stream,
                       q, emb_rel_k, relq, H, D, T, ld, in_bs, scale, nrel);
  }
  const int DT = cdiv(D, 32);
  const long blocks = (long)cdiv(T, 128) * H;
  (void)B;
  int nsplit = 1;
  static const int max_split = std::min(8, getenv("RVCX_ATT_MAXSPLIT") ? atoi(getenv("RVCX_ATT_MAXSPLIT")) : 8);
  static const int want_blocks = getenv("RVCX_ATT_BLOCKS") ? atoi(getenv("RVCX_ATT_BLOCKS")) : 200;
  static const int min_keys = getenv("RVCX_ATT_MINKEYS") ? atoi(getenv("RVCX_ATT_MINKEYS")) : 256;
  while (nsplit < max_split && blocks * nsplit < want_blocks && T / (nsplit * 2) >= min_keys) nsplit *= 2;
  float* opart = nullptr;
  if (nsplit > 1) {
    if (split_scratch) opart = split_scratch;
    else nsplit = 1;
  }
  float* mo = nsplit > 1 ? nullptr : mb;
  float* lo = nsplit > 1 ? nullptr : lb;
  dim3 grid(cdiv(T, 128) * nsplit, H, B);
  static const int h3_env = getenv("RVCX_ATT_H3") ? atoi(getenv("RVCX_ATT_H3")) : 1;
  const int h3 = h3_env && !g_force_fp32 && allow_h3;
  if (h3) {
    RVCX_CHECK(split_scratch != nullptr, "attention: the split-fp16 kernel needs its scratch");
    const int ntile = cdiv(T, 32);
    uint4* kimg = reinterpret_cast<uint4*>(split_scratch + (size_t)B * H * 8 * 98 * T);
    uint4* vimg = kimg + (size_t)B * H * ntile * (DT * 256);
    const dim3 pg(ntile, H, B);
    if (DT == 1) {
      hipLaunchKernelGGL(att_presplit_kernel<1>, pg, dim3(256), 0, stream, k, v, kimg, vimg, H, D, T, ld, in_bs, lens, ovf, ovf_layer, seq);
      hipLaunchKernelGGL(attn_h3_kernel<1>, grid, dim3(256), 0, stream, q, kimg, vimg, out, mo, lo, relq, H, D, T, ld, in_bs,
                         out_bs, scale, window, lens, nsplit, opart, ovf, ovf_layer, seq);
    } else if (DT == 2) {
      hipLaunchKernelGGL(att_presplit_kernel<2>, pg, dim3(256), 0, stream, k, v, kimg, vimg, H, D, T, ld, in_bs, lens, ovf, ovf_layer, seq);
      hipLaunchKernelGGL(attn_h3_kernel<2>, grid, dim3(256), 0, stream, q, kimg, vimg, out, mo, lo, relq, H, D, T, ld, in_bs,
                         out_bs, scale, window, lens, nsplit, opart, ovf, ovf_layer, seq);
    } else {
      hipLaunchKernelGGL(att_presplit_kernel<3>, pg, dim3(256), 0, stream, k, v, kimg, vimg, H, D, T, ld, in_bs, lens, ovf, ovf_layer, seq);
      hipLaunchKernelGGL(attn_h3_kernel<3>, grid, dim3(256), 0, stream, q, kimg, vimg, out, mo, lo, relq, H, D, T, ld, in_bs,
                         out_bs, scale, window, lens, nsplit, opart, ovf, ovf_layer, seq);
    }
  }
  else if (DT == 1)
    hipLaunchKernelGGL(attn_kernel<1>, grid, dim3(256), 0, stream, q, k, v, out, mo, lo, relq, H, D, T, ld, in_bs,
                       out_bs, scale, window, lens, nsplit, opart);
  else if (DT == 2)
    hipLaunchKernelGGL(attn_kernel<2>, grid, dim3(256), 0, stream, q, k, v, out, mo, lo, relq, H, D, T, ld, in_bs,
                       out_bs, scale, window, lens, nsplit, opart);
  else
    hipLaunchKernelGGL(attn_kernel<3>, grid, dim3(256), 0, stream, q, k, v, out, mo, lo, relq, H, D, T, ld, in_bs,
                       out_bs, scale, window, lens, nsplit, opart);
  if (nsplit > 1)
    hipLaunchKernelGGL(attn_merge_kernel, dim3(cdiv(T, 64), H * 4, B), dim3(256), 0, stream, opart, out, mb, lb, H, D,
                       32 * DT, T, ld, out_bs, nsplit, lens);
  if (emb_rel_v) {
    size_t lds = ((size_t)nrel * D + 32 * (nrel + 1) + (size_t)D * 32 + (size_t)D * (32 + 2 * window)) * sizeof(float);
    hipLaunchKernelGGL(rel_values_kernel, dim3(cdiv(T, 32), H, B), dim3(256), lds, stream, q, k, relq, mb, lb,
                       emb_rel_v, out, H, D, T, ld, in_bs, out_bs, scale, window, lens);
  }
  RVCX_HIP(hipGetLastError());
}

size_t attention_scratch_floats(int B, int H, int T, int window) {
  return (size_t)B * H * T * (2 * window + 1) + 2 * (size_t)B * H * T;
}

size_t attention_split_floats(int B, int H, int T) { return (size_t)B * H * (8 * 98 * (size_t)T + 2 * 96 * ((size_t)T + 32)); }

double attention_flops(int B, int H, int D, int T) { return 4.0 * B * H * (double)T * T * D; }

}
```

### polgen-rvc_amd/csrc/ctx.h

```cpp
#pragma once
#include <memory>

#include "common.h"
#include "conv.h"
#include "gemm.h"

namespace rvcx {

struct SynthModel;
struct RmvpeModel;
struct FcpeModel;
struct CrepeModel;
struct HubertModel;
struct IndexData;

class WeightRegion {
 public:
  static constexpr size_t kChunkBytes = (size_t)32 << 20;
  static constexpr int kMaxFlags = 4096;
  static constexpr size_t kHeaderBytes = kMaxFlags;
  WeightRegion() {
    flags_.reset(new uint8_t[kMaxFlags]);
    std::memset(flags_.get(), 0, kMaxFlags);
  }
// ... 70 lines not shown
      t += region + ": layer " + std::to_string(i) + " of " + std::to_string(nflags_) + " (" +
           ((size_t)i < desc_.size() && !desc_[i].empty() ? desc_[i] : std::string("?")) + ")\n";
    return t;
  }
  void seal() {
    if (chunks_.empty()) reserve(256);
    RVCX_HIP(hipMemcpy(chunks_[0].base, flags_.get(), kMaxFlags, hipMemcpyHostToDevice));
  }
  void adopt() {
    if (chunks_.empty()) return;
    RVCX_HIP(hipMemcpy(flags_.get(), chunks_[0].base, kMaxFlags, hipMemcpyDeviceToHost));
  }
  int n_chunks() const { return (int)chunks_.size(); }
  void* chunk_base(int i) const { return chunks_[i].base; }
  size_t chunk_used(int i) const { return chunks_[i].off; }
  size_t used() const {
    size_t t = 0;
    for (auto& c : chunks_) t += c.off;
    return t;
  }
  uint64_t layout_hash() const { return hash_; }

 private:
  struct Chunk {
    void* base;
    size_t cap, off;
  };
  void new_chunk(size_t bytes) {
    Chunk c{nullptr, bytes, 0};
    RVCX_HIP(hipMalloc(&c.base, bytes));
    chunks_.push_back(c);
  }
  void mix(uint64_t v) {
    for (int i = 0; i < 8; ++i) {
      hash_ ^= (v >> (8 * i)) & 0xff;
      hash_ *= 1099511628211ull;
    }
  }
  std::vector<Chunk> chunks_;
  std::unique_ptr<uint8_t[]> flags_;
  int* ovf_words_ = nullptr;
  int nflags_ = 0, dropped_ = 0;
  std::vector<int> pinned_;
  std::vector<std::string> desc_;
  uint64_t hash_ = 1469598103934665603ull;
};

class WeightSlab {
 public:
  float* upload(const std::vector<float>& h) { return cur().upload(h); }
  float* upload(const float* h, size_t n) { return cur().upload(h, n); }
  uint8_t* new_flag(bool v) { return cur().new_flag(v); }
  WeightRegion& cur() {
    if (!cur_) fail("internal: weight upload outside a RegionScope");
    return *cur_;
  }
  WeightRegion* cur_ = nullptr;
};

struct StageTimer {
  hipEvent_t ev[16];
  bool made = false;
  void make() {
    if (made) return;
    for (auto& e : ev) RVCX_HIP(hipEventCreate(&e));
    made = true;
  }
};

struct Ctx {
  int device = 0;
  hipStream_t stream = nullptr;
  hipStream_t stream2 = nullptr;
  hipEvent_t ev_hub = nullptr;
  hipEvent_t ev_syn[2] = {nullptr, nullptr};
  hipEvent_t ev_hubdone[2] = {nullptr, nullptr};
  hipStream_t aux[2] = {nullptr, nullptr};
  hipEvent_t ev_aux[6] = {nullptr, nullptr, nullptr, nullptr, nullptr, nullptr};
  hipEvent_t ev_fork = nullptr, ev_join = nullptr;
  hipStream_t stream_io = nullptr;
  hipEvent_t ev_io = nullptr;
  hipEvent_t ev_front[2] = {nullptr, nullptr};
  hipEvent_t ev_done[2] = {nullptr, nullptr};
  hipEvent_t ev_src[2] = {nullptr, nullptr};
  Arena arena;
  size_t arena_budget = 0;
  Arena arena_f0;
  Arena arena_hub;
  WeightSlab slab;
  std::string last_error;
  double flops = 0.0;
  int resblock_streams = 0;
  bool serial = false;
  bool serial_env = false;
  int* dev_err = nullptr;
  int* err_host = nullptr;
  bool err_snapshot = false;
  void snapshot_dev_err(hipStream_t s);
  void check_dev_err();
  bool take_overflow();
  long fp32_reruns = 0;
  long gru_fallbacks = 0;
  bool inject_gru_timeout = false;
  int64_t kmeans_exhaustive = 0;
  struct TicketSlot {
    Arena arena;
    int* err = nullptr;
    int* err_host = nullptr;
    char* stage = nullptr;
    size_t stage_cap = 0;
  } slot[2];
  int* err_words = nullptr;
  int* err_words_host = nullptr;
  int launch_seq = 0;
  float timing[9] = {0};
  std::vector<int> last_mbs;
  std::vector<std::vector<long>> last_cuts;
  StageTimer timer;
  std::unique_ptr<HubertModel> hubert;
  std::unique_ptr<RmvpeModel> rmvpe;
  std::unique_ptr<FcpeModel> fcpe;
  std::unique_ptr<CrepeModel> crepe;
  std::vector<std::unique_ptr<SynthModel>> synths;
  std::unique_ptr<IndexData> index;
  Ctx();
  ~Ctx();
  float* splitk_buf[4] = {nullptr, nullptr, nullptr, nullptr};
  static constexpr long kSplitKFloats = 32L << 20;
  int splitk_items = 1;
  void ensure_splitk(int items) {
    if (items <= splitk_items) return;
    RVCX_HIP(hipDeviceSynchronize());
    for (auto& p : splitk_buf)
      if (p) {
        (void)hipFree(p);
        p = nullptr;
      }
    splitk_items = items;
  }
  void pair_on(const PairArgs& a, hipStream_t s) {
    const double f = 2.0 * 2.0 * a.B * (double)a.C * a.C * a.k * a.T;
    flops += f;
    PairArgs b = a;
    b.ovf = dev_err;
    b.seq = ++launch_seq;
    conv_launch_pair(b, f, s);
  }
  void block3_on(const Block3Args& a, hipStream_t s) {
    const double f = 3.0 * 2.0 * 2.0 * a.B * (double)a.C * a.C * 3 * a.T;
    flops += f;
    Block3Args b = a;
    b.ovf = dev_err;
    b.seq = ++launch_seq;
    conv_launch_block3(b, f, s);
  }
  void gemm_on(GemmArgs a, hipStream_t s) {
    const double f = 2.0 * (double)a.rows * a.cout * a.cin;
    flops += f;
    a.ovf = dev_err;
    a.seq = ++launch_seq;
    {
      const int si = (s == stream2) ? 1 : (s == aux[0] ? 2 : (s == aux[1] ? 3 : 0));
      if (!splitk_buf[si]) RVCX_HIP(hipMalloc(&splitk_buf[si], kSplitKFloats * splitk_items * sizeof(float)));
      a.part = splitk_buf[si];
      a.part_cap = kSplitKFloats * splitk_items;
    }
    conv_launch_gemm(a, f, s);
// ... 80 lines not shown
```

### polgen-rvc_amd/csrc/ops.h

```cpp
#pragma once
#include "common.h"

namespace rvcx {

void launch_attention(const float* q, const float* k, const float* v, float* out, int B, int H, int D, int T,
                      int ld, long in_bs, long out_bs, float scale, const float* emb_rel_k, const float* emb_rel_v, int window,
                      const int* lens, float* scratch, float* split_scratch, hipStream_t stream,
                      int* ovf = nullptr ,
                      int* ovf_layer = nullptr, int seq = 0 ,
                      bool allow_h3 = true );
size_t attention_scratch_floats(int B, int H, int T, int window);
size_t attention_split_floats(int B, int H, int T);
double attention_flops(int B, int H, int D, int T);

size_t bigru_scratch_bytes(int B);
int bigru_probe_publish();
int bigru_probe_state();
void launch_bigru(const float* gi, const float* whh, const float* bhh, float* y, int B, int T, int H,
                  void* scratch, int* err, hipStream_t stream, const int* lens = nullptr);

void launch_layernorm_c(const float* x, const float* gamma, const float* beta, float* y, int B, int C, int T,
                        float eps, const int* lens, hipStream_t s);
void launch_layernorm_tm(const float* x, long ld_x, const float* gamma, const float* beta, float* y, long ld_y, void* ys,
                         long ld_ys, long rows, int C, float eps, int* ovf, int* ovf_next, int seq, hipStream_t s);
void launch_cf_to_tm(const float* x, long x_bs, float* y, long ld_y, void* ys, long ld_ys, int B, int C, int T, int* ovf,
                     int* ovf_next, int seq, hipStream_t s);
void launch_groupnorm_gelu(const float* x, const float* gamma, const float* beta, float* y, int B, int C, int T,
                           float eps, hipStream_t s, const int* lens = nullptr);
size_t hubert_conv0_part_doubles(int B, int C, int T);
void launch_hubert_conv0_gn_gelu_split(const float* wav, long wav_bs, const float* w, int K, int stride, int Cp, const float* gamma,
                                       const float* beta, double* part, float* stats, void* y_split, int B, int C, int T,
                                       float eps, hipStream_t s, const int* lens, int* ovf, int* ovf_layer, int seq);
void launch_groupnorm_gelu_split(const float* x, const float* gamma, const float* beta, float* stats, void* y_split, int B,
                                 int C, int T, float eps, hipStream_t s, const int* lens, int* ovf, int* ovf_layer, int seq);
void launch_transpose(const float* x, float* y, int B, int R, int Cc, hipStream_t s);
void launch_embed_pitch(float* x, const float* emb, const int* pitch, int B, int C, int T, float scale,
                        float slope, const int* lens, hipStream_t s);
void launch_sample_z(const float* stats, const float* noise, float* z, int B, int C, int T, const int* lens,
                     hipStream_t s);
void launch_flip_channels(const float* x, float* y, int B, int C, int T, hipStream_t s);
void launch_wn_gate(const float* a, const float* g, int goff, int gstride, float* acts, int B, int H, int T,
                    hipStream_t s);
void launch_wn_res_skip(float* x, float* out, const float* rs, int B, int H, int T, int last, int first,
                        const int* lens, hipStream_t s);
void launch_coupling_sub(float* x, const float* m, int B, int half, int T, const int* lens, hipStream_t s);
void launch_mask(float* x, int B, int C, int T, const int* lens, hipStream_t s);
void launch_add_channel_bias(float* x, const float* g, int B, int C, int T, hipStream_t s);
void launch_sine_source(const float* f0, const float* noise, float* har, int B, int T, int upp, float sr,
                        const float* lin_wb, const int* lens, double* scratch, hipStream_t s);
void launch_randn(float* out, size_t n, uint64_t seed, uint64_t offset, hipStream_t s);

void launch_reflect_pad(const float* x, float* y, int B, int n, int p, long y_bs, hipStream_t s, const int* ns = nullptr,
                        long x_bs = 0);
int* dev_ints(Arena& A, const int* v, int n, hipStream_t s);
void set_dev_ints(int* dst, const int* v, int n, hipStream_t s);
inline int* dev_ints(Arena& A, const std::vector<int>& v, hipStream_t s) { return dev_ints(A, v.data(), (int)v.size(), s); }
std::vector<int*> dev_ints_many(Arena& A, const std::vector<std::vector<int>>& vs, hipStream_t s);
void launch_magnitude(const float* ft, float* mag, int B, int nb, int F, hipStream_t s, float eps = 0.f);
void launch_mel_post(const float* mel, float* out, int B, int nmel, int F, int Tp, const float* bn,
                     hipStream_t s, const int* fs = nullptr, const int* tps = nullptr);
void launch_log_clamp(const float* x, float* y, long n, float floor, hipStream_t s);
void launch_avgpool2(const float* x, float* y, int planes, int H, int Wp, long x_ps, long y_ps, hipStream_t s);
void launch_copy_strided(const float* x, float* y, int B, long n, long x_bs, long y_bs, hipStream_t s);
void launch_gru_input(const float* x, float* y, int B, int Cc, int T, int Wp, hipStream_t s);
void launch_decode_f0(const float* sal, float* f0, int B, int T, int ld, float thred, float f0_min, float f0_max,
                      hipStream_t s);
void launch_f0_coarse(const float* f0_in, float* f0_out, int* coarse, int n, double pitch, double f0_min,
                      double f0_max, hipStream_t s);

void launch_f0_override(const double* rep, int count, int start, float* f0, int* coarse, int n, double f0_min,
                        double f0_max, hipStream_t s);
std::vector<double> f0_file_track(const float* tbl, int rows);

struct ResampleFilter {
  const double* win = nullptr;
  const double* delta = nullptr;
  double scale = 1.0, time_increment = 1.0;
  int index_step = 512;
  int table = 512, nwin = 0, exact = 0;
};
long resample_out_len(long n, int sr_in, int sr_out);
int resample_default_kind();
ResampleFilter make_resample_filter(Arena& A, int sr_in, int sr_out, hipStream_t s, int kind = -1);
void launch_resample_f64(const ResampleFilter& f, const double* x, long n, int channels, double* y, long n_out,
                         hipStream_t s);
void launch_resample_f32(const ResampleFilter& f, const float* x, long n, float* y, long n_out, hipStream_t s);
size_t resample_table_doubles(int kind);
// ... 24 lines not shown
```

### polgen-rvc_amd/csrc/resblock.hip

```cpp
#include <algorithm>
#include <cstdlib>
#include <mutex>
#include <type_traits>

#include "conv.h"
#include "conv_device.h"
#include "h3_device.h"

namespace rvcx {

namespace {

constexpr int kPairHalo = 64;
constexpr int kPairPadY = 16;
#ifndef RVCX_PAIR_SCHED_FENCE
#define RVCX_PAIR_SCHED_FENCE 0
#endif
constexpr bool kSchedFence = RVCX_PAIR_SCHED_FENCE != 0;
#ifndef RVCX_PAIR_PIPE
#define RVCX_PAIR_PIPE 1
#endif
constexpr bool kPipe = RVCX_PAIR_PIPE != 0;
#ifndef RVCX_PAIR_ABL
#define RVCX_PAIR_ABL 0
// ... 964 lines not shown
    static_assert(THREADS / 64 * 32 * P * 4 <= Y1_ELEMS * 16, "staging tiles must fit the Y1 region");
    __syncthreads();
    float* stg = reinterpret_cast<float*>(lds) + wave * (32 * P);
    const int lr = lane >> 3, lc = (lane & 7) * 4;
#pragma unroll
    for (int m = 0; m < WM; ++m)
#pragma unroll
      for (int n = 0; n < WN; ++n) {
#pragma unroll
        for (int r = 0; r < 16; ++r) stg[((r & 3) + 8 * (r >> 2) + 4 * h) * P + i] = acc[m][n][r] * inv;
        __builtin_amdgcn_wave_barrier();
        const int col0 = wc * (WN * 32) + n * 32 + lc;
        const int pos0 = n0 + col0;
        const bool ok = col0 < BN_OUT && pos0 < a.T;
        float4 v[4], rv[4], pv[4];
#pragma unroll
        for (int p = 0; p < 4; ++p) {
          const int co = wr * (WM * 32) + m * 32 + lr + 8 * p;
          const long off = (long)b * a.bs + (long)co * a.cs + pos0;
          v[p] = *reinterpret_cast<const float4*>(stg + (lr + 8 * p) * P + lc);
          rv[p] = ok ? *reinterpret_cast<const float4*>(a.x + off) : make_float4(0.f, 0.f, 0.f, 0.f);
          pv[p] = (ok && a.acc2_mode != ACC2_NONE && a.acc2_mode != ACC2_SET) ? *reinterpret_cast<const float4*>(a.y2 + off)
                                                                              : make_float4(0.f, 0.f, 0.f, 0.f);
        }
        __builtin_amdgcn_wave_barrier();
        if (ok) {
#pragma unroll
          for (int p = 0; p < 4; ++p) {
            const int co = wr * (WM * 32) + m * 32 + lr + 8 * p;
            const long off = (long)b * a.bs + (long)co * a.cs + pos0;
            const float bb = a.b2 ? a.b2[co] : 0.f;
            float o[4] = {v[p].x + bb + rv[p].x, v[p].y + bb + rv[p].y, v[p].z + bb + rv[p].z, v[p].w + bb + rv[p].w};
#pragma unroll
            for (int q = 0; q < 4; ++q) o[q] = pos0 + q < len ? o[q] : 0.f;
            if (a.y) *reinterpret_cast<float4*>(a.y + off) = make_float4(o[0], o[1], o[2], o[3]);
            if (a.acc2_mode != ACC2_NONE) {
              const float pp[4] = {pv[p].x, pv[p].y, pv[p].z, pv[p].w};
#pragma unroll
              for (int q = 0; q < 4; ++q) {
                if (a.acc2_mode == ACC2_ADD) o[q] = pp[q] + o[q];
                else if (a.acc2_mode == ACC2_ADD_DIV) o[q] = (pp[q] + o[q]) / a.acc2_div;
              }
              *reinterpret_cast<float4*>(a.y2 + off) = make_float4(o[0], o[1], o[2], o[3]);
            }
          }
        }
      }
  }
  stamp(5);
}

template <int C, int NT, int WR, int WC, int K, int KKT, int NCS, bool EARLY>
__global__ __launch_bounds__(64 * WR * WC) void resblock_pair_persist_kernel(const PairArgs a) {
  constexpr int THREADS = 64 * WR * WC;
  constexpr int N1 = 32 * NT, N1P = N1 + kPairPadY, WROW = N1 + kPairHalo;
  constexpr int WM = (C / 32) / WR, WN = NT / WC;
  constexpr int NCHUNK = C / 16;
  constexpr int NG = (K + KKT - 1) / KKT;
  constexpr int SL = NCS * KKT;
  constexpr int A_ELEMS = SL * 4 * C, NA = (A_ELEMS + THREADS - 1) / THREADS;
  constexpr int B_TASKS = NCS * 2 * WROW, NBT = (B_TASKS + THREADS - 1) / THREADS;
  constexpr int BN_OUT = (N1 - (K - 1)) & ~3, H2 = (K - 1) / 2;
  static_assert(WM >= 1 && WN >= 1 && WM * WR * 32 == C && WN * WC == NT, "bad tile");
  static_assert(NCS == 1 || KKT == K, "several chunks per stage only with all taps resident");
  static_assert(NCHUNK % NCS == 0, "chunk sets must tile the channels");
  extern __shared__ uint4 lds[];
  constexpr int Y1_ELEMS = NCHUNK * 4 * N1P;
  uint4* Y1 = lds;
  uint4* As = Y1 + Y1_ELEMS;
  uint4* Bs = As + A_ELEMS;
  float* bias_s = reinterpret_cast<float*>(Bs + NCS * 4 * WROW);

  int tid = threadIdx.x, lane = tid & 63, wave = tid >> 6;
  int wr = wave / WC, wc = wave % WC;
  int i = lane & 31, h = lane >> 5;
  const int b = blockIdx.z;
  const int pad1 = (K - 1) * a.dil / 2;
  const int len = a.lens ? a.lens[b] : a.T;
  const int wuse = N1 + (K - 1) * a.dil;
  const float slope = a.slope;
  const H3Rsrc xr = h3_rsrc(a.x + (long)b * a.bs, C * a.cs * 4);
  const H3Rsrc w1r = h3_rsrc(a.w1, K * NCHUNK * 4 * C * 16);
  const H3Rsrc w2r = h3_rsrc(a.w2, K * NCHUNK * 4 * C * 16);
  const int xrow = a.cs * 4;
  constexpr int slab = 4 * C * 16;

  int first, count;
  {
    const int nt = (a.T + BN_OUT - 1) / BN_OUT, nwg = gridDim.x, w = blockIdx.x;
    if (a.xcd_order && nwg >= 8) {
      const int x = w & 7, j = w >> 3;
      const int q = nt >> 3, r = nt & 7;
      const int x0 = x * q + (x < r ? x : r), xn = q + (x < r ? 1 : 0);
      const int m = (nwg >> 3) + (x < (nwg & 7) ? 1 : 0);
      const int q2 = xn / m, r2 = xn % m;
      first = x0 + j * q2 + (j < r2 ? j : r2);
      count = q2 + (j < r2 ? 1 : 0);
    } else {
      const int q = nt / nwg, r = nt % nwg;
      first = w * q + (w < r ? w : r);
      count = q + (w < r ? 1 : 0);
    }
  }
  if (count <= 0) return;
  const int ntiles_all = (a.T + BN_OUT - 1) / BN_OUT;
  int cur_tile = first;
  auto stamp = [&](int k) {
    if (a.trace && tid == 0) a.trace[((long)b * ntiles_all + cur_tile) * 8 + k] = (long long)wall_clock64();
  };

  f32x16 acc[WM][WN];
  auto zero_acc = [&]() {
#pragma unroll
    for (int m = 0; m < WM; ++m)
#pragma unroll
      for (int n = 0; n < WN; ++n)
#pragma unroll
        for (int r = 0; r < 16; ++r) acc[m][n][r] = 0.f;
  };

  int a_cl[NA], a_kkl[NA], a_off[NA];
  int b_off[NBT], b_row[NBT];
  int lr = 0, lc = 0;
  auto derive_thread = [&]() {
    int t0 = threadIdx.x;
#if defined(__HIP_DEVICE_COMPILE__)
    asm volatile("" : "+v"(t0));
#endif
    tid = t0;
    lane = tid & 63;
    wave = tid >> 6;
    wr = wave / WC;
    wc = wave % WC;
    i = lane & 31;
    h = lane >> 5;
    lr = lane >> 3;
    lc = (lane & 7) * 4;
#pragma unroll
    for (int j = 0; j < NA; ++j) {
      const int e = tid + THREADS * j;
      const int co = e % C, rest = e / C;
      const int slot = rest / 4;
      a_cl[j] = slot / KKT;
      a_kkl[j] = slot % KKT;
      a_off[j] = e < A_ELEMS ? ((rest % 4) * C + co) * 16 : kH3Oob;
    }
#pragma unroll
    for (int j = 0; j < NBT; ++j) {
      const int t = tid + THREADS * j;
      const int ch2 = t / WROW;
      b_row[j] = (ch2 >> 1) * 16 + (ch2 & 1) * 8;
    }
  };
  derive_thread();
  auto set_input_tile = [&](int tile) {
    const int in_base = tile * BN_OUT - H2 - pad1;
#pragma unroll
    for (int j = 0; j < NBT; ++j) {
      const int t = tid + THREADS * j;
      const int ch2 = t / WROW, p = t - ch2 * WROW;
      const int pos = in_base + p;
      b_off[j] = (t < B_TASKS && p < wuse && pos >= 0 && pos < len) ? pos * 4 : kH3Oob;
    }
  };

  uint4 ra[NA];
// ... 107 lines not shown

  for (int ti = 0; ti < count; ++ti) {
    const int tile = first + ti;
    cur_tile = tile;
    const int n0 = tile * BN_OUT;
    const bool has_next = ti + 1 < count;
    if (ti > 0) derive_thread();
    stamp(0);
    zero_acc();
    for (int chunk = 0; chunk < NCHUNK; chunk += NCS) {
#pragma unroll
      for (int g = 0; g < NG; ++g) {
        const bool last_stage = chunk + NCS >= NCHUNK && g == NG - 1;
        __syncthreads();
        if (g == 0 && chunk > 0) commit_b();
        commit_a();
        __syncthreads();
        if (chunk == 0 && g == 0) stamp(1);
        if (!last_stage) fetch_a(w1r, g + 1 == NG ? chunk + NCS : chunk, g + 1 == NG ? 0 : (g + 1) * KKT);
        else fetch_a(w2r, 0, 0);
        if (g == 0 && chunk + NCS < NCHUNK) {
          fetch_b(chunk + NCS);
        } else if (EARLY && g == 0 && has_next) {
          set_input_tile(tile + 1);
          fetch_b(0);
        }
        if (NG > 1 && g == NG - 1) compute(Last{}, Bs, WROW, 4 * WROW, g * KKT, a.dil);
        else compute(Full{}, Bs, WROW, 4 * WROW, g * KKT, a.dil);
      }
    }
    stamp(2);
    if (!EARLY && has_next) {
      set_input_tile(tile + 1);
      fetch_b(0);
    }
#pragma unroll
    for (int m = 0; m < WM; ++m)
#pragma unroll
      for (int n = 0; n < WN; ++n) {
        const int c_t = wr * (WM * 32) + m * 32;
        const int j = wc * (WN * 32) + n * 32 + i;
        const int pos1 = n0 - H2 + j;
        const bool live = pos1 >= 0 && pos1 < len;
#pragma unroll
        for (int g = 0; g < 4; ++g) {
          typedef _Float16 half4 __attribute__((ext_vector_type(4)));
          const int cg = c_t + 8 * g;
          half4 hi, lo;
          const float4 bq = *reinterpret_cast<const float4*>(bias_s + cg + 4 * h);
          const float b4[4] = {bq.x, bq.y, bq.z, bq.w};
#pragma unroll
          for (int q = 0; q < 4; ++q) {
            float v = acc[m][n][4 * g + q] * inv + b4[q];
            v = fmaxf(v, v * slope);
            v = live ? v : 0.f;
            ovf |= !(fabsf(v) < kH3ActLimit);
            const _Float16 vh = (_Float16)v;
            hi[q] = vh;
            lo[q] = (_Float16)((v - (float)vh) * kH3Scale);
          }
          char* e_hi = reinterpret_cast<char*>(Y1 + (((cg >> 4) * 2 + 0) * 2 + (g & 1)) * N1P + j) + 8 * h;
          char* e_lo = reinterpret_cast<char*>(Y1 + (((cg >> 4) * 2 + 1) * 2 + (g & 1)) * N1P + j) + 8 * h;
          *reinterpret_cast<half4*>(e_hi) = hi;
          *reinterpret_cast<half4*>(e_lo) = lo;
        }
      }

    zero_acc();
    stamp(3);
    uint4 rv[WM][WN][4];
    auto request_res = [&](int n) {
#pragma unroll
      for (int m = 0; m < WM; ++m) {
        const int col0 = wc * (WN * 32) + n * 32 + lc;
        const int pos0 = n0 + col0;
        const bool ok = col0 < BN_OUT && pos0 < a.T;
#pragma unroll
        for (int p = 0; p < 4; ++p) {
          const int co = wr * (WM * 32) + m * 32 + lr + 8 * p;
          rv[m][n][p] = h3_load4(xr, ok ? (co * a.cs + pos0) * 4 : kH3Oob);
        }
      }
    };
    if (EARLY && NG == 1) request_res(0);
    for (int chunk = 0; chunk < NCHUNK; chunk += NCS) {
#pragma unroll
      for (int g = 0; g < NG; ++g) {
        const bool last_stage = chunk + NCS >= NCHUNK && g == NG - 1;
        __syncthreads();
        commit_a();
        if (last_stage && has_next) commit_b();
        __syncthreads();
        if (!last_stage) fetch_a(w2r, g + 1 == NG ? chunk + NCS : chunk, g + 1 == NG ? 0 : (g + 1) * KKT);
        else if (has_next) fetch_a(w1r, 0, 0);
        if (EARLY ? (NG > 1 && g == 0 && chunk + NCS >= NCHUNK) : last_stage) request_res(0);
        if (NG > 1 && g == NG - 1) compute(Last{}, Y1 + chunk * 4 * N1P, N1P, 4 * N1P, g * KKT, 1);
        else compute(Full{}, Y1 + chunk * 4 * N1P, N1P, 4 * N1P, g * KKT, 1);
      }
    }
    stamp(4);
    {
      constexpr int P = 36;
      static_assert(THREADS / 64 * 32 * P * 4 <= NCHUNK * 4 * N1P * 16, "staging tiles must fit the Y1 region");
      __syncthreads();
      float* stg = reinterpret_cast<float*>(lds) + wave * (32 * P);
#pragma unroll
      for (int n = 1; n < WN; ++n) request_res(n);
#pragma unroll
      for (int n = 0; n < WN; ++n)
#pragma unroll
        for (int m = 0; m < WM; ++m) {
#pragma unroll
          for (int r = 0; r < 16; ++r) stg[((r & 3) + 8 * (r >> 2) + 4 * h) * P + i] = acc[m][n][r] * inv;
          __builtin_amdgcn_wave_barrier();
          const int col0 = wc * (WN * 32) + n * 32 + lc;
          const int pos0 = n0 + col0;
          const bool ok = col0 < BN_OUT && pos0 < a.T;
          float4 v[4], pv[4];
#pragma unroll
          for (int p = 0; p < 4; ++p) {
            const int co = wr * (WM * 32) + m * 32 + lr + 8 * p;
            const long off = (long)b * a.bs + (long)co * a.cs + pos0;
            v[p] = *reinterpret_cast<const float4*>(stg + (lr + 8 * p) * P + lc);
            pv[p] = (ok && a.acc2_mode != ACC2_NONE && a.acc2_mode != ACC2_SET) ? *reinterpret_cast<const float4*>(a.y2 + off)
                                                                                : make_float4(0.f, 0.f, 0.f, 0.f);
          }
          __builtin_amdgcn_wave_barrier();
          if (ok) {
#pragma unroll
            for (int p = 0; p < 4; ++p) {
              const int co = wr * (WM * 32) + m * 32 + lr + 8 * p;
              const long off = (long)b * a.bs + (long)co * a.cs + pos0;
              const float bb = bias_s[C + co];
              const float4 rr = __builtin_bit_cast(float4, rv[m][n][p]);
              float o[4] = {v[p].x + bb + rr.x, v[p].y + bb + rr.y, v[p].z + bb + rr.z, v[p].w + bb + rr.w};
#pragma unroll
              for (int q = 0; q < 4; ++q) o[q] = pos0 + q < len ? o[q] : 0.f;
              if (a.y) *reinterpret_cast<float4*>(a.y + off) = make_float4(o[0], o[1], o[2], o[3]);
              if (a.acc2_mode != ACC2_NONE) {
                const float pp[4] = {pv[p].x, pv[p].y, pv[p].z, pv[p].w};
#pragma unroll
                for (int q = 0; q < 4; ++q) {
                  if (a.acc2_mode == ACC2_ADD) o[q] = pp[q] + o[q];
                  else if (a.acc2_mode == ACC2_ADD_DIV) o[q] = (pp[q] + o[q]) / a.acc2_div;
                }
                *reinterpret_cast<float4*>(a.y2 + off) = make_float4(o[0], o[1], o[2], o[3]);
              }
            }
          }
        }
    }
    stamp(5);
  }
  if (ovf) report_h3_overflow(a.ovf, a.ovf_layer, a.seq);
}

struct PairCfg {
  int C, K, n1, threads, variant, bn_out;
  bool wide;
  size_t lds;
  void (*kern)(const PairArgs);
  bool persist = false;
  int per_cu = 1;
};
template <int C, int NT, int WR, int WC, int K, int KKT, int NCS, int V = 0, bool TRIM = false, int RESPF = 0, bool OVL = false>
constexpr PairCfg make_cfg() {
  constexpr size_t y1 = (size_t)(C / 16) * 4 * (32 * NT + pair_pady(K, TRIM)), as = (size_t)NCS * KKT * 4 * C,
                   bs = (size_t)NCS * 4 * (32 * NT + pair_halo(K, TRIM));
  return {C, K, 32 * NT, 64 * WR * WC, V, RESPF == 3 ? ((32 * NT - (K - 1)) & ~3) : 32 * NT - (K - 1), RESPF == 3,
          (OVL ? (y1 > bs ? y1 : bs) + as : y1 + as + bs) * 16,
          resblock_pair_kernel<C, NT, WR, WC, K, KKT, NCS, TRIM, RESPF, OVL>};
}
template <int C, int NT, int WR, int WC, int K, int KKT, int NCS, bool EARLY = true, int V = 10, int PER_CU = 1>
constexpr PairCfg make_persist() {
  constexpr size_t y1 = (size_t)(C / 16) * 4 * (32 * NT + kPairPadY), as = (size_t)NCS * KKT * 4 * C,
                   bs = (size_t)NCS * 4 * (32 * NT + kPairHalo);
  return {C, K, 32 * NT, 64 * WR * WC, V, (32 * NT - (K - 1)) & ~3, true, (y1 + as + bs) * 16 + 2 * C * 4,
          resblock_pair_persist_kernel<C, NT, WR, WC, K, KKT, NCS, EARLY>, true, PER_CU};
}
template <int C, int NT, int WR, int WC, int K, int G, int V, bool OVL = false>
constexpr PairCfg make_adir() {
  constexpr size_t y1 = (size_t)(C / 16) * 4 * (32 * NT + kPairPadY), bs = (size_t)2 * 4 * (32 * NT + kPairHalo);
  return {C, K, 32 * NT, 64 * WR * WC, V, (32 * NT - (K - 1)) & ~3, true, (OVL ? y1 : y1 + bs) * 16,
          resblock_pair_adir_kernel<C, NT, WR, WC, K, G, OVL>};
}
template <int C, int NT, int WR, int WC, int K, int G, int V>
constexpr PairCfg make_sp() {
  constexpr size_t y1 = (size_t)(C / 16) * 4 * (32 * NT + kPairPadY), bs2 = (size_t)2 * 4 * (32 * NT + kPairHalo),
                   as = (size_t)2 * G * 4 * C;
  return {C, K, 32 * NT, 64 * WR * WC, V, (32 * NT - (K - 1)) & ~3, true, ((y1 > bs2 ? y1 : bs2) + as) * 16 + 64,
          resblock_pair_sp_kernel<C, NT, WR, WC, K, G>};
}
const PairCfg kPair[] = {
    make_cfg<32, 16, 1, 8, 3, 3, 2, 0, false, 2>(),  make_cfg<32, 16, 1, 8, 7, 7, 1, 0, false, 2>(),  make_cfg<32, 16, 1, 8, 11, 11, 1, 0, false, 2>(),
    make_cfg<64, 8, 2, 4, 3, 3, 2, 0, false, 2>(),   make_cfg<64, 8, 2, 4, 7, 7, 1, 0, false, 2>(),   make_cfg<64, 8, 2, 4, 11, 11, 1, 0, false, 2>(),
    make_cfg<128, 6, 4, 3, 3, 3, 1, 0, false, 2>(),  make_cfg<128, 4, 4, 2, 7, 7, 1, 0, false, 2>(),  make_cfg<128, 6, 4, 3, 11, 4, 1, 0, false, 1>(),
    make_cfg<256, 3, 4, 3, 3, 2, 1, 0, false, 1>(),  make_cfg<256, 3, 4, 3, 7, 2, 1, 0, false, 1>(),  make_cfg<256, 3, 4, 3, 11, 2, 1, 0, false, 1>(),
    make_cfg<128, 4, 4, 2, 3, 3, 2, 1>(),  make_cfg<128, 6, 4, 3, 7, 4, 1, 1>(),  make_cfg<128, 4, 4, 2, 11, 6, 1, 1>(),
    make_cfg<32, 8, 1, 4, 3, 3, 2, 2, true>(),   make_cfg<32, 8, 1, 4, 7, 7, 1, 2, true>(),   make_cfg<32, 8, 1, 4, 11, 11, 1, 2, true>(),
    make_cfg<64, 4, 2, 2, 3, 3, 2, 2, true>(),   make_cfg<64, 4, 2, 2, 7, 7, 1, 2, true>(),   make_cfg<64, 4, 2, 2, 11, 4, 1, 2, true>(),
    make_cfg<128, 3, 2, 3, 3, 2, 1, 2, true>(),  make_cfg<128, 3, 2, 3, 7, 2, 1, 2, true>(),  make_cfg<128, 3, 2, 3, 11, 2, 1, 2, true>(),
    make_cfg<32, 16, 1, 8, 3, 3, 2, 4, false, 3>(),  make_cfg<32, 16, 1, 8, 7, 7, 1, 4, false, 3>(),  make_cfg<32, 16, 1, 8, 11, 11, 1, 4, false, 3>(),
    make_cfg<64, 8, 2, 4, 3, 3, 2, 4, false, 3>(),   make_cfg<64, 8, 2, 4, 7, 7, 1, 4, false, 3>(),   make_cfg<64, 8, 2, 4, 11, 11, 1, 4, false, 3>(),
    make_cfg<128, 6, 4, 3, 3, 3, 1, 4, false, 3>(),  make_cfg<128, 4, 4, 2, 7, 7, 1, 4, false, 3>(),  make_cfg<128, 6, 4, 3, 11, 4, 1, 4, false, 3>(),
    make_cfg<256, 3, 4, 3, 3, 2, 1, 4, false, 3>(),  make_cfg<256, 3, 4, 3, 7, 2, 1, 4, false, 3>(),  make_cfg<256, 3, 4, 3, 11, 2, 1, 4, false, 3>(),
    make_cfg<32, 32, 1, 8, 3, 3, 2, 5, false, 3, true>(),  make_cfg<32, 32, 1, 8, 7, 7, 1, 5, false, 3, true>(),  make_cfg<32, 32, 1, 8, 11, 11, 1, 5, false, 3, true>(),
    make_cfg<64, 16, 1, 8, 3, 3, 2, 5, false, 3, true>(),  make_cfg<64, 16, 1, 8, 7, 3, 1, 5, false, 3, true>(),  make_cfg<64, 16, 1, 8, 11, 4, 1, 5, false, 3, true>(),
    make_cfg<128, 8, 2, 4, 3, 3, 1, 5, false, 3, true>(),  make_cfg<128, 8, 2, 4, 7, 3, 1, 5, false, 3, true>(),  make_cfg<128, 8, 2, 4, 11, 3, 1, 5, false, 3, true>(),
    make_adir<32, 16, 1, 8, 3, 3, 6>(),  make_adir<32, 16, 1, 8, 7, 4, 6>(),  make_adir<32, 16, 1, 8, 11, 4, 6>(),
    make_adir<64, 8, 2, 4, 3, 3, 6>(),   make_adir<64, 8, 2, 4, 7, 4, 6>(),   make_adir<64, 8, 2, 4, 11, 4, 6>(),
    make_adir<128, 6, 4, 3, 3, 3, 6>(),  make_adir<128, 6, 4, 3, 7, 2, 6>(),  make_adir<128, 6, 4, 3, 11, 2, 6>(),
    make_adir<32, 16, 1, 8, 3, 3, 7>(),  make_adir<32, 16, 1, 8, 7, 4, 7>(),  make_adir<32, 16, 1, 8, 11, 4, 7>(),
    make_adir<64, 16, 1, 8, 3, 2, 7, true>(),  make_adir<64, 16, 1, 8, 7, 2, 7, true>(),  make_adir<64, 16, 1, 8, 11, 2, 7, true>(),
    make_adir<128, 8, 2, 4, 3, 2, 7, true>(),  make_adir<128, 8, 2, 4, 7, 2, 7, true>(),  make_adir<128, 8, 2, 4, 11, 2, 7, true>(),
    make_sp<32, 16, 1, 8, 3, 3, 8>(),  make_sp<32, 16, 1, 8, 7, 4, 8>(),  make_sp<32, 16, 1, 8, 11, 4, 8>(),
    make_sp<64, 8, 2, 4, 3, 3, 8>(),   make_sp<64, 8, 2, 4, 7, 4, 8>(),   make_sp<64, 8, 2, 4, 11, 4, 8>(),
    make_sp<128, 6, 4, 3, 3, 3, 8>(),  make_sp<128, 6, 4, 3, 7, 3, 8>(),  make_sp<128, 6, 4, 3, 11, 3, 8>(),
    make_persist<32, 16, 1, 8, 3, 3, 2, false>(),  make_persist<32, 16, 1, 8, 7, 7, 1, false>(),  make_persist<32, 16, 1, 8, 11, 11, 1, false>(),
    make_persist<64, 8, 2, 4, 3, 3, 2, false>(),   make_persist<64, 8, 2, 4, 7, 7, 1, false>(),   make_persist<64, 8, 2, 4, 11, 11, 1, false>(),
    make_persist<128, 6, 4, 3, 3, 3, 1, false>(),  make_persist<128, 6, 4, 2, 7, 4, 1, false>(),  make_persist<128, 6, 4, 2, 11, 4, 1, false>(),
    make_persist<32, 16, 1, 8, 3, 3, 2, true, 11>(),  make_persist<32, 16, 1, 8, 7, 7, 1, true, 11>(),  make_persist<32, 16, 1, 8, 11, 11, 1, true, 11>(),
    make_persist<64, 8, 2, 4, 3, 3, 2, true, 11>(),   make_persist<64, 8, 2, 4, 7, 7, 1, true, 11>(),   make_persist<64, 8, 2, 4, 11, 11, 1, true, 11>(),
    make_persist<128, 6, 4, 3, 11, 4, 1, false, 11>(),  make_persist<128, 4, 4, 2, 7, 7, 1, false, 11>(),
    make_persist<128, 6, 4, 2, 3, 3, 1, false, 13>(),
    make_cfg<32, 16, 1, 8, 3, 3, 2, 3>(),  make_cfg<32, 16, 1, 8, 7, 7, 1, 3>(),  make_cfg<32, 16, 1, 8, 11, 11, 1, 3>(),
    make_cfg<64, 8, 2, 4, 3, 3, 2, 3>(),   make_cfg<64, 8, 2, 4, 7, 7, 1, 3>(),   make_cfg<64, 8, 2, 4, 11, 11, 1, 3>(),
    make_cfg<128, 6, 4, 3, 3, 3, 1, 3>(),  make_cfg<128, 4, 4, 2, 7, 7, 1, 3>(),  make_cfg<128, 6, 4, 3, 11, 4, 1, 3>(),
};
constexpr int kPairBase = 12;
bool pair_aligned(const PairArgs& a) {
  auto al = [](const void* p) { return (reinterpret_cast<uintptr_t>(p) & 15) == 0; };
  return a.cs % 4 == 0 && a.T % 4 == 0 && a.bs % 4 == 0 && al(a.x) && al(a.y) && al(a.y2);
}
// ... 83 lines not shown
```

### polgen-rvc_amd/csrc/synth.hip

```cpp
#include <algorithm>
#include <cmath>
#include <cstdlib>

#include "models.h"
#include "ops.h"

namespace rvcx {

std::vector<float> wn_weight(const TensorTable& t, const std::string& p, int dim) {
  if (t.has(p + ".weight")) return t.f32(p + ".weight");
  std::string gn = p + ".parametrizations.weight.original0", vn = p + ".parametrizations.weight.original1";
  if (!t.has(gn)) {
    gn = p + ".weight_g";
    vn = p + ".weight_v";
  }
  std::vector<float> g = t.f32(gn), v = t.f32(vn);
  const auto shp = t.shape(vn);
  RVCX_CHECK(shp.size() == 3, "weight-norm tensor must be 3-D: " + p);
  const int64_t d0 = shp[0], d1 = shp[1], d2 = shp[2];
  std::vector<float> w(v.size());
  if (dim == 0) {
    RVCX_CHECK((int64_t)g.size() == d0, "weight_g shape: " + p);
    for (int64_t a = 0; a < d0; ++a) {
      double ss = 0.0;
// ... 148 lines not shown
  size_t mx = 0, sum = (size_t)B * T * cf.up_initial_channel;
  long tt = T;
  for (size_t i = 0; i < m.stages.size(); ++i) {
    tt *= cf.up_rates[i];
    const size_t n = (size_t)B * tt * m.stages[i].ch;
    mx = std::max(mx, n);
    sum += n + 1024;
  }
  return (enc + dec + 2 * sum + 9 * mx) * sizeof(float) + ((size_t)64 << 20);
}

namespace {

struct Timer3 {
  Ctx& c;
  hipEvent_t* e;
  Timer3(Ctx& cc, hipEvent_t* ev) : c(cc), e(ev) {}
  void mark(int i) {
    if (e) RVCX_HIP(hipEventRecord(e[i], c.stream));
  }
};

int* upload_ints(Ctx& c, const std::vector<int>& v) {
  int* d = c.arena.alloc<int>(v.size());
  RVCX_HIP(hipMemcpyAsync(d, v.data(), v.size() * sizeof(int), hipMemcpyHostToDevice, c.stream));
  return d;
}

}

void synth_forward(Ctx& c, const SynthModel& m, const SynthIO& io, hipEvent_t* stage_ev) {
  const auto& cf = m.cfg;
  const int B = io.B, T = io.T, hid = cf.hidden_channels, inter = cf.inter_channels, filt = cf.filter_channels;
  const int heads = cf.n_heads, kc = hid / heads, half = inter / 2, gin = cf.gin_channels;
  hipStream_t s = c.stream;
  Arena& A = c.arena;
  Timer3 tm(c, stage_ev);
  tm.mark(0);
  const int head = io.skip_head, Tk = T - head;
  RVCX_CHECK(head >= 0 && Tk > 0, "synth: skip_head outside [0, T)");
  if (head > 0) {
    RVCX_CHECK(io.dec_skip == 0, "synth: dec_skip and skip_head exclude each other");
    if (io.lens_host)
      for (int b = 0; b < B; ++b) RVCX_CHECK(io.lens_host[b] == T, "synth: skip_head needs equal lengths (every item T frames)");
  }

  bool ragged = false;
  if (io.lens_host)
    for (int b = 0; b < B; ++b) ragged |= io.lens_host[b] != T;
  std::vector<const int*> lens_stage(m.stages.size() + 2, nullptr);
  const int* lens = nullptr;
  if (ragged) {
    std::vector<int> l(io.lens_host, io.lens_host + B);
    lens = upload_ints(c, l);
    lens_stage[0] = lens;
    for (size_t i = 0; i < m.stages.size(); ++i) {
      for (auto& x : l) x *= cf.up_rates[i];
      lens_stage[i + 1] = upload_ints(c, l);
    }
  }
  std::vector<int> sidv(io.sid_host, io.sid_host + B);

  const long Tupp = (long)Tk * m.upp;
  const float* pitchf = io.pitchf;
  if (head > 0) {
    float* pf = A.alloc<float>((size_t)B * Tk);
    launch_copy_strided(io.pitchf + head, pf, B, Tk, T, Tk, s);
    pitchf = pf;
  }
  float* har = A.alloc<float>((size_t)B * Tupp);
  std::vector<float*> nz(m.stages.size(), nullptr);
  std::vector<char> nz_fused(m.stages.size(), 0);
  for (size_t i = 0; i < m.stages.size(); ++i) {
    const auto& S = m.stages[i];
    ConvArgs probe = convT1d_args(S.up, nullptr, nullptr, 1, 1, cf.up_rates[i]);
    probe.pre_act = ACT_LRELU;
    probe.pre_slope = 0.1f;
    static const bool fuse_on = !getenv("RVCX_NOISE_FUSE") || atoi(getenv("RVCX_NOISE_FUSE")) != 0;
    static const int fuse_max_k = getenv("RVCX_NOISE_FUSE_K") ? atoi(getenv("RVCX_NOISE_FUSE_K")) : 4;
    nz_fused[i] = fuse_on && S.noise.cin == 1 && S.noise.groups == 1 && S.noise.k >= 1 && S.noise.cout == S.ch &&
                  S.noise.k <= fuse_max_k;
    (void)probe;
  }
  {
    hipStream_t sn = c.serial ? s : c.aux[0];
    if (sn != s) {
      RVCX_HIP(hipEventRecord(c.ev_src[0], s));
      RVCX_HIP(hipStreamWaitEvent(sn, c.ev_src[0], 0));
    }
    double* sc = A.alloc<double>((size_t)B * Tk * 2);
    launch_sine_source(pitchf, io.src_noise, har, B, Tk, m.upp, (float)cf.sr, m.lin_wb, lens, sc, sn);
    long tt = Tk;
    for (size_t i = 0; i < m.stages.size(); ++i) {
      const auto& S = m.stages[i];
      tt *= cf.up_rates[i];
      if (nz_fused[i]) continue;
      nz[i] = A.alloc<float>((size_t)B * S.ch * tt);
      static const bool dense_on = !getenv("RVCX_NOISE_DENSE") || atoi(getenv("RVCX_NOISE_DENSE")) != 0;
      if (dense_on && S.noise_dense_cin > 0 && Tupp == tt * S.noise_stride) {
        const int sp = S.noise_dense_cin, st = S.noise_stride;
        float* x2 = A.alloc<float>((size_t)B * sp * tt);
        RVCX_HIP(hipMemsetAsync(x2, 0, (size_t)B * sp * tt * sizeof(float), sn));
        for (int b = 0; b < B; ++b) launch_transpose(har + (size_t)b * Tupp, x2 + (size_t)b * sp * tt, 1, (int)tt, st, sn);
        ConvArgs a = conv1d_args(S.noise_dense, x2, nz[i], B, (int)tt, (int)tt, 1, 1, 1);
        a.lens_out = lens_stage[i + 1];
        c.conv_on(a, sn);
        continue;
      }
      ConvArgs a = conv1d_args(S.noise, har, nz[i], B, (int)Tupp, (int)tt, S.noise_stride, 1, S.noise_pad);
      a.lens_in = lens_stage[m.stages.size()];
      a.lens_out = lens_stage[i + 1];
      c.conv_on(a, sn);
    }
    if (sn != s) RVCX_HIP(hipEventRecord(c.ev_src[1], sn));
  }

  float* x = A.alloc<float>((size_t)B * hid * T);
  {
    ConvArgs a = conv1d_args(m.emb_phone, io.phone_ct, x, B, T, T);
    a.lens_out = lens;
    c.conv(a);
    launch_embed_pitch(x, m.emb_pitch, io.pitch, B, hid, T, std::sqrt((float)hid), 0.1f, lens, s);
  }
  float* qkv = A.alloc<float>((size_t)B * 3 * hid * T);
  float* att = A.alloc<float>((size_t)B * hid * T);
  float* tmp = A.alloc<float>((size_t)B * hid * T);
  float* hbuf = A.alloc<float>((size_t)B * filt * T);
  float* scratch = A.alloc<float>(attention_scratch_floats(B, heads, T, 10));
  float* asplit = A.alloc<float>(attention_split_floats(B, heads, T));
  const float scale = 1.f / std::sqrt((float)kc);
  for (const auto& L : m.enc) {
    ConvArgs a = conv1d_args(L.qkv, x, qkv, B, T, T);
    a.lens_out = lens;
    c.conv(a);
    launch_attention(qkv, qkv + (size_t)hid * T, qkv + (size_t)2 * hid * T, att, B, heads, kc, T, T,
                     (long)3 * hid * T, (long)hid * T, scale, L.rel_k, L.rel_v, 10, lens, scratch, asplit, s, c.dev_err, L.att.word,
                     ++c.launch_seq, L.att.h3());
    c.flops += attention_flops(B, heads, kc, T);
    a = conv1d_args(L.o, att, tmp, B, T, T);
    a.lens_out = lens;
    conv_set_res(a, x, hid, T);
    c.conv(a);
    launch_layernorm_c(tmp, L.g1, L.b1, x, B, hid, T, 1e-5f, nullptr, s);
    const int k = L.ffn1.k, pl = (k - 1) / 2;
    a = conv1d_args(L.ffn1, x, hbuf, B, T, T, 1, 1, pl);
    a.act = ACT_RELU;
    a.lens_in = lens;
    a.lens_out = lens;
    c.conv(a);
    a = conv1d_args(L.ffn2, hbuf, tmp, B, T, T, 1, 1, pl);
    a.lens_in = lens;
    a.lens_out = lens;
    conv_set_res(a, x, hid, T);
    c.conv(a);
    launch_layernorm_c(tmp, L.g2, L.b2, x, B, hid, T, 1e-5f, nullptr, s);
  }
  float* stats = io.stats_out ? io.stats_out : A.alloc<float>((size_t)B * 2 * inter * T);
  {
    launch_mask(x, B, hid, T, lens, s);
    ConvArgs a = conv1d_args(m.proj, x, stats, B, T, T);
    a.lens_out = lens;
    c.conv(a);
  }
  tm.mark(1);

  float* z = A.alloc<float>((size_t)B * inter * T);
  float* z2 = A.alloc<float>((size_t)B * inter * T);
  launch_sample_z(stats, io.z_noise, z, B, inter, T, lens, s);
  if (head > 0) {
    launch_copy_strided(z + head, z2, B * inter, Tk, T, Tk, s);
    std::swap(z, z2);
  }
  float* g = A.alloc<float>((size_t)B * gin);
  for (int b = 0; b < B; ++b)
    RVCX_HIP(hipMemcpyAsync(g + (size_t)b * gin, m.emb_g + (size_t)sidv[b] * gin, gin * sizeof(float),
                            hipMemcpyDeviceToDevice, s));
  {
    float* h = att;
    float* xin = qkv;
    float* acts = tmp;
    float* rs = hbuf;
    RVCX_CHECK(filt >= 2 * hid, "buffer reuse assumes filter_channels >= 2*hidden");
    float* wout = A.alloc<float>((size_t)B * hid * T);
    float* mbuf = A.alloc<float>((size_t)B * half * T);
    float* gc = A.alloc<float>((size_t)B * 6 * hid);
    for (int f = 3; f >= 0; --f) {
      const auto& F = m.flows[f];
      launch_flip_channels(z, z2, B, inter, Tk, s);
      std::swap(z, z2);
      ConvArgs a = conv1d_args(F.pre, z, h, B, Tk, Tk);
      a.x_bs = (long)inter * Tk;
      a.lens_out = lens;
      c.conv(a);
      a = conv1d_args(F.cond, g, gc, B, 1, 1);
      c.conv(a);
      for (int i = 0; i < 3; ++i) {
        a = conv1d_args(F.in_l[i], h, xin, B, Tk, Tk, 1, 1, (F.in_l[i].k - 1) / 2);
        a.lens_in = lens;
        a.lens_out = lens;
        c.conv(a);
        launch_wn_gate(xin, gc, i * 2 * hid, 6 * hid, acts, B, hid, Tk, s);
        a = conv1d_args(F.rs_l[i], acts, rs, B, Tk, Tk);
        a.lens_out = lens;
        c.conv(a);
        launch_wn_res_skip(h, wout, rs, B, hid, Tk, i == 2, i == 0, lens, s);
      }
      a = conv1d_args(F.post, wout, mbuf, B, Tk, Tk);
      a.lens_out = lens;
      c.conv(a);
      launch_coupling_sub(z, mbuf, B, half, Tk, lens, s);
    }
  }
  if (io.z_out)
    RVCX_HIP(hipMemcpyAsync(io.z_out, z, (size_t)B * inter * Tk * sizeof(float), hipMemcpyDeviceToDevice, s));
  tm.mark(2);
  if (io.ev_decoder) RVCX_HIP(hipEventRecord(io.ev_decoder, s));

  if (!c.serial) RVCX_HIP(hipStreamWaitEvent(s, c.ev_src[1], 0));
  static const int dec_batch_env = getenv("RVCX_DEC_BATCH") ? std::max(1, atoi(getenv("RVCX_DEC_BATCH"))) : 8;
  bool equal_lens = true;
  if (io.lens_host)
    for (int b = 1; b < B; ++b) equal_lens &= io.lens_host[b] == io.lens_host[0];
  const int dec_batch = equal_lens ? dec_batch_env : 1;
  const int C0 = cf.up_initial_channel;
  const size_t dec_mark = A.mark();
  for (int b0 = 0; b0 < B; b0 += dec_batch) {
    const int db = std::min(dec_batch, B - b0);
    A.reset(dec_mark);
    const bool own = io.lens_host != nullptr && (db == 1 || equal_lens);
    const int Tfull = own ? io.lens_host[b0] - head : Tk;
    RVCX_CHECK(Tfull > 0 && Tfull <= Tk, "synth: item length outside (0, T]");
    const int skip = (io.dec_skip > 0 && (own || !lens) && Tfull - 2 * io.dec_skip > 2 * m.dec_rf_frames) ? io.dec_skip : 0;
    const int Td = Tfull - 2 * skip;
    float* cur = A.alloc<float>((size_t)db * C0 * Td);
    {
      ConvArgs a = conv1d_args(m.conv_pre, z + (size_t)b0 * inter * Tk + skip, cur, db, Td, Td, 1, 1, 3);
      a.x_bs = (long)inter * Tk;
      a.x_cs = Tk;
      a.lens_in = (lens && !own) ? lens + b0 : nullptr;
      c.conv(a);
      float* gcond = A.alloc<float>((size_t)db * C0);
      a = conv1d_args(m.cond, g + (size_t)b0 * gin, gcond, db, 1, 1);
      c.conv(a);
      launch_add_channel_bias(cur, gcond, db, C0, Td, s);
    }
    long Tin = Td, Tin_c = Tk, off = skip;
    for (size_t i = 0; i < m.stages.size(); ++i) {
      const auto& S = m.stages[i];
      const long Tout = Tin * cf.up_rates[i], Tout_c = Tin_c * cf.up_rates[i];
      off *= cf.up_rates[i];
      const size_t n = (size_t)db * S.ch * Tout;
      float* xs = A.alloc<float>(n);
      const size_t stage_mark = A.mark();
      float* xu = A.alloc<float>(n);
      const int nk = cf.n_resblocks;
      float* xcb[4];
      float* xtb[4];
      for (int j = 0; j < nk; ++j) {
        xcb[j] = A.alloc<float>(n);
        xtb[j] = A.alloc<float>(n);
      }
      const int* lin = (lens_stage[i] && !own) ? lens_stage[i] + b0 : nullptr;
      const int* lout = (lens_stage[i + 1] && !own) ? lens_stage[i + 1] + b0 : nullptr;
      ConvArgs a = convT1d_args(S.up, cur, xu, db, (int)Tin, (int)Tout);
      a.pre_act = ACT_LRELU;
      a.pre_slope = 0.1f;
      a.lens_in = lin;
      a.lens_out = lout;
      if (nz_fused[i]) {
        a.nz_har = har + (size_t)b0 * Tupp + (size_t)skip * m.upp;
        a.nz_bs = Tupp;
        a.nz_w = S.noise.w;
        a.nz_wstride = S.noise.cin_gp * S.noise.cout_gp;
        a.nz_b = S.noise.bias;
        a.nz_k = S.noise.k;
        a.nz_stride = S.noise_stride;
        a.nz_pad = S.noise_pad;
        a.nz_len = (own || skip) ? (int)((long)Td * m.upp) : (int)Tupp;
        a.nz_lens = (lens_stage[m.stages.size()] && !own) ? lens_stage[m.stages.size()] + b0 : nullptr;
      } else {
        conv_set_res(a, nz[i] + (size_t)b0 * S.ch * Tout_c + off, S.ch, (int)Tout_c);
      }
      c.conv(a);
      const int side = c.serial ? 0 : c.resblock_streams;
      hipStream_t rs[4] = {s, side ? c.aux[0] : s, side == 1 ? c.aux[1] : s, s};
      RVCX_HIP(hipEventRecord(c.ev_aux[0], s));
      for (int j = 1; j < nk && j < 3; ++j) RVCX_HIP(hipStreamWaitEvent(rs[j], c.ev_aux[0], 0));
      for (int j = 0; j < nk; ++j) {
        hipStream_t sj = rs[j];
        const int k = cf.res_kernels[j];
        const float* xin = xu;
        float* xc = xcb[j];
        float* xt = xtb[j];
        if (k == 3) {
          Block3Args ba;
          ba.x = xu;
          ba.y = nullptr;
          ba.y2 = xs;
          bool ok3 = true;
          for (int mi = 0; mi < 3; ++mi) {
            const auto &L1 = S.c1[j][mi], &L2 = S.c2[j][mi];
            ba.w1[mi] = (L1.w_h3 && L1.h3_ok && *L1.h3_ok) ? L1.w_h3 : nullptr;
            ba.w2[mi] = (L2.w_h3 && L2.h3_ok && *L2.h3_ok) ? L2.w_h3 : nullptr;
            ba.b1[mi] = L1.bias;
            ba.b2[mi] = L2.bias;
            ba.dil[mi] = cf.res_dilations[j][mi];
            ok3 = ok3 && L1.cin == S.ch && L1.cout == S.ch && L1.k == 3 && L2.cin == S.ch && L2.cout == S.ch && L2.k == 3;
          }
          ba.ovf_layer = S.c1[j][0].ovf_word;
          ba.lens = lout;
          ba.B = db;
          ba.C = S.ch;
          ba.T = (int)Tout;
          ba.bs = (long)S.ch * Tout;
          ba.cs = (int)Tout;
          ba.slope = 0.1f;
          ba.acc2_mode = j == 0 ? ACC2_SET : (j == nk - 1 ? ACC2_ADD_DIV : ACC2_ADD);
          ba.acc2_div = (float)nk;
          if (nk == 1) ba.acc2_mode = ACC2_SET;
          if (ok3 && resblock3_ok(ba)) {
            if (j > 0) RVCX_HIP(hipStreamWaitEvent(sj, c.ev_aux[j], 0));
            c.block3_on(ba, sj);
            RVCX_HIP(hipEventRecord(c.ev_aux[j + 1], sj));
            continue;
          }
        }
        for (int mi = 0; mi < 3; ++mi) {
// ... 100 lines not shown
```

Baseline: 1249.

## Fold attention rel-logits into presplit, merge rel terms, prefetch resblock sums, hoist conds

Merges the relative-logits kernel into the K/V presplit launch as extra blocks and adds a merge kernel that applies the relative-position terms in the split-K reduction. It also moves the speaker-conditioning convs for the flows and decoder onto the auxiliary stream ahead of time, and prefetches the accumulate-sum operand in the fused resblock pair kernel through buffer loads. The aim is fewer launches and less serial latency on the main stream, at the cost of more complex kernels and extra cross-stream events.

```diff
diff --git a/include/rvcx.h b/include/rvcx.h
--- a/include/rvcx.h
+++ b/include/rvcx.h
@@ -281,6 +281,9 @@
 int rvcx_op_resblock_pair(rvcx_ctx*, const float* x, const float* w1, const float* b1, const float* w2,
                           const float* b2, float* y, int B, int C, int T, int K, int dil, float slope, int fused,
                           const int32_t* lens);
+int rvcx_op_resblock_pair_sum(rvcx_ctx*, const float* x, const float* w1, const float* b1, const float* w2,
+                              const float* b2, float* y2, int B, int C, int T, int K, int dil, float slope, int mode,
+                              float div, const int32_t* lens);
 int rvcx_op_resblock3(rvcx_ctx*, const float* x, const float* w1, const float* b1, const float* w2, const float* b2,
                       float* y, int B, int C, int T, const int32_t* dils, float slope, const int32_t* lens);
 int rvcx_bench_resblock_pair(rvcx_ctx*, int B, int C, int T, int K, int dil, int fused, int iters,
@@ -288,6 +291,7 @@
 int rvcx_bench_conv1d(rvcx_ctx*, int B, int Cin, int Tin, int Cout, int K, int stride, int dil, int groups,
                       int iters, float* ms_per_launch);
 int rvcx_conv_override(int tile, int variant, int splitk);
+int rvcx_att_fold_override(int fold);
 int rvcx_op_convtranspose1d(rvcx_ctx*, const float* x, const float* w, const float* bias, float* y,
                             int B, int Cin, int Tin, int Cout, int K, int stride, int pad,
                             int pre_lrelu, float pre_slope);
diff --git a/polgen-rvc_amd/_lib.py b/polgen-rvc_amd/_lib.py
--- a/polgen-rvc_amd/_lib.py
+++ b/polgen-rvc_amd/_lib.py
@@ -155,6 +155,7 @@
     "rvcx_op_groupnorm_gelu", "rvcx_op_hubert_conv0", "rvcx_op_sine_source", "rvcx_op_randn", "rvcx_op_reflect_pad",
     "rvcx_op_mel_post", "rvcx_op_decode_f0", "rvcx_op_avgpool2", "rvcx_op_gru_input", "rvcx_op_upsample_protect",
     "rvcx_kmeans", "rvcx_ivf_assign", "rvcx_kmeans_exhaustive", "rvcx_index_features",
+    "rvcx_op_resblock_pair_sum", "rvcx_att_fold_override",
     "rvcx_op_resblock3", "rvcx_flac_encode_bound", "rvcx_flac_encode_s16", "rvcx_flac_info", "rvcx_flac_decode_s32", "rvcx_flac_last_error",
 ]
 
@@ -690,6 +691,25 @@
                  "op_resblock_pair")
         return y
 
+    def resblock_pair_sum(self, x, w1, b1, w2, b2, y2, mode, div=1.0, dil=1, slope=0.1, lens=None):
+        x, w1, w2 = f32(x), f32(w1), f32(w2)
+        B, Cc, T = x.shape
+        K = w1.shape[2]
+        out = np.array(y2, dtype=np.float32, order="C", copy=True)
+        assert out.shape == x.shape
+        b1 = None if b1 is None else f32(b1)
+        b2 = None if b2 is None else f32(b2)
+        li = i32(lens)
+        self._ck(lib().rvcx_op_resblock_pair_sum(self._h, _p(x), _p(w1), _p(b1), _p(w2), _p(b2), _p(out), B, Cc, T, K, dil,
+                                                 C.c_float(slope), int(mode), C.c_float(div), _p(li, C.c_int32)),
+                 "op_resblock_pair_sum")
+        return out
+
+    @staticmethod
+    def att_fold_override(fold=True):
+        if lib().rvcx_att_fold_override(1 if fold else 0) != 0:
+            raise RvcxError("att_fold_override: " + (lib().rvcx_last_error(None) or b"").decode())
+
     def resblock3(self, x, w1, b1, w2, b2, dils=(1, 3, 5), slope=0.1, lens=None):
         x, w1, w2 = f32(x), f32(w1), f32(w2)
         B, Cc, T = x.shape
diff --git a/polgen-rvc_amd/csrc/api_ops.hip b/polgen-rvc_amd/csrc/api_ops.hip
--- a/polgen-rvc_amd/csrc/api_ops.hip
+++ b/polgen-rvc_amd/csrc/api_ops.hip
@@ -118,6 +118,45 @@
   API_END
 }
 
+int rvcx_op_resblock_pair_sum(rvcx_ctx* ctx, const float* x, const float* w1, const float* b1, const float* w2,
+                              const float* b2, float* y2, int B, int Cc, int T, int K, int dil, float slope, int mode,
+                              float div, const int32_t* lens) {
+  API_BEGIN(ctx)
+  TEMP_REGION(C);
+  if (mode != ACC2_SET && mode != ACC2_ADD && mode != ACC2_ADD_DIV) fail("resblock pair sum: mode must be 1 (set), 2 (add) or 3 (add, divide)");
+  const size_t n = (size_t)B * Cc * T;
+  C->arena.reserve(n * 4 * 3 + (64 << 20));
+  C->arena.reset();
+  ConvW L1 = make_conv(*C, w1, b1, Cc, Cc, K, 1, true);
+  ConvW L2 = make_conv(*C, w2, b2, Cc, Cc, K, 1, true);
+  float* dx = to_dev(*C, x, n);
+  float* dy2 = to_dev(*C, y2, n);
+  PairArgs pa;
+  pa.x = dx;
+  pa.y = nullptr;
+  pa.y2 = dy2;
+  pa.acc2_mode = mode;
+  pa.acc2_div = div;
+  pa.w1 = (L1.w_h3 && *L1.h3_ok) ? L1.w_h3 : nullptr;
+  pa.w2 = (L2.w_h3 && *L2.h3_ok) ? L2.w_h3 : nullptr;
+  pa.b1 = L1.bias;
+  pa.b2 = L2.bias;
+  pa.lens = (lens ? to_dev(*C, lens, B) : nullptr);
+  pa.B = B;
+  pa.C = Cc;
+  pa.T = T;
+  pa.bs = (long)Cc * T;
+  pa.cs = T;
+  pa.k = K;
+  pa.dil = dil;
+  pa.slope = slope;
+  if (!resblock_pair_ok(pa)) fail("resblock pair sum: shape not supported by the fused kernel");
+  C->pair_on(pa, C->stream);
+  to_host(*C, y2, dy2, n);
+  C->arena.reset();
+  API_END
+}
+
 int rvcx_op_resblock3(rvcx_ctx* ctx, const float* x, const float* w1, const float* b1, const float* w2, const float* b2,
                       float* y, int B, int Cc, int T, const int32_t* dils, float slope, const int32_t* lens) {
   API_BEGIN(ctx)
@@ -257,6 +296,12 @@
   return 0;
 }
 
+int rvcx_att_fold_override(int fold) {
+  REQUIRE_DEBUG(nullptr, "rvcx_att_fold_override")
+  rvcx::g_att_fold = fold != 0 ? 1 : 0;
+  return 0;
+}
+
 int rvcx_bench_conv1d(rvcx_ctx* ctx, int B, int Cin, int Tin, int Cout, int K, int stride, int dil, int groups,
                       int iters, float* ms_per_launch) {
   REQUIRE_DEBUG(ctx, "rvcx_bench_conv1d")
diff --git a/polgen-rvc_amd/csrc/attention.hip b/polgen-rvc_amd/csrc/attention.hip
--- a/polgen-rvc_amd/csrc/attention.hip
+++ b/polgen-rvc_amd/csrc/attention.hip
@@ -5,6 +5,8 @@
 #include "ops.h"
 
 namespace rvcx {
+
+int g_att_fold = 1;
 
 constexpr int KT = 32;
 constexpr int VROW = 33;
@@ -187,20 +189,20 @@
 constexpr int kAttOob = 0x7ffffff0;
 
 template <int DT>
-__global__ __launch_bounds__(256) void att_presplit_kernel(const float* __restrict__ k, const float* __restrict__ v,
-                                                           uint4* __restrict__ kimg, uint4* __restrict__ vimg, int H, int D,
-                                                           int T, int ld, long in_bs, const int* lens, int* ovf_word,
-                                                           int* ovf_layer, int seq) {
+__device__ __forceinline__ void att_presplit_body(const float* __restrict__ k, const float* __restrict__ v,
+                                                  uint4* __restrict__ kimg, uint4* __restrict__ vimg, int H, int D, int T,
+                                                  int ld, long in_bs, const int* lens, int* ovf_word, int* ovf_layer,
+                                                  int seq, int kt, int ntile) {
   constexpr int NS = 2 * DT;
   constexpr int K_ELEMS = NS * 2 * 32, V_ELEMS = DT * 2 * 2 * 32;
-  const int kt = blockIdx.x, hd = blockIdx.y, b = blockIdx.z, tid = threadIdx.x;
+  const int hd = blockIdx.y, b = blockIdx.z, tid = threadIdx.x;
   const int len = lens ? lens[b] : T;
   const int k0 = kt * 32;
   const long base = (long)b * in_bs + (long)hd * D * ld;
   const float* kb = k + base;
   const float* vb = v + base;
-  uint4* ko = kimg + (((long)b * H + hd) * gridDim.x + kt) * (2 * K_ELEMS);
-  uint4* vo = vimg + (((long)b * H + hd) * gridDim.x + kt) * (2 * V_ELEMS);
+  uint4* ko = kimg + (((long)b * H + hd) * ntile + kt) * (2 * K_ELEMS);
+  uint4* vo = vimg + (((long)b * H + hd) * ntile + kt) * (2 * V_ELEMS);
   bool ovf = false;
   for (int e0 = tid; e0 < K_ELEMS; e0 += 256) {
     const int key = e0 & 31, hh = (e0 >> 5) & 1, s = e0 >> 6;
@@ -235,6 +237,13 @@
     vo[(((dt * 2 + s2) * 2 + 1) * 2 + hh) * 32 + dd] = __builtin_bit_cast(uint4, a2);
   }
   if (ovf) report_h3_overflow(ovf_word, ovf_layer, seq);
+}
+template <int DT>
+__global__ __launch_bounds__(256) void att_presplit_kernel(const float* __restrict__ k, const float* __restrict__ v,
+                                                           uint4* __restrict__ kimg, uint4* __restrict__ vimg, int H, int D,
+                                                           int T, int ld, long in_bs, const int* lens, int* ovf_word,
+                                                           int* ovf_layer, int seq) {
+  att_presplit_body<DT>(k, v, kimg, vimg, H, D, T, ld, in_bs, lens, ovf_word, ovf_layer, seq, blockIdx.x, gridDim.x);
 }
 
 typedef unsigned att_u32x4 __attribute__((ext_vector_type(4)));
@@ -477,15 +486,14 @@
   }
 }
 
-__global__ __launch_bounds__(256) void rel_logits_kernel(const float* __restrict__ q, const float* __restrict__ ek,
-                                                         float* __restrict__ relq, int H, int D, int T, int ld,
-                                                         long in_bs, float scale, int nrel) {
-  extern __shared__ float eks[];
+__device__ __forceinline__ void rel_logits_body(const float* __restrict__ q, const float* __restrict__ ek,
+                                                float* __restrict__ relq, int H, int D, int T, int ld, long in_bs,
+                                                float scale, int nrel, int qblk, float* eks ) {
   for (int idx = threadIdx.x; idx < nrel * D; idx += 256) eks[idx] = ek[idx];
   __syncthreads();
   const int tq = threadIdx.x & 63, part = __builtin_amdgcn_readfirstlane(threadIdx.x >> 6);
   const int nmine = part < nrel ? (nrel - part + 3) / 4 : 0;
-  const int t = blockIdx.x * 64 + tq;
+  const int t = qblk * 64 + tq;
   const int hd = blockIdx.y, b = blockIdx.z;
   if (t >= T) return;
   const float* qb = q + (long)b * in_bs + (long)hd * D * ld;
@@ -529,6 +537,24 @@
     const int r = part + 4 * i;
     if (r < nrel) o[r] = acc[i];
   }
+}
+__global__ __launch_bounds__(256) void rel_logits_kernel(const float* __restrict__ q, const float* __restrict__ ek,
+                                                         float* __restrict__ relq, int H, int D, int T, int ld,
+                                                         long in_bs, float scale, int nrel) {
+  extern __shared__ float eks[];
+  rel_logits_body(q, ek, relq, H, D, T, ld, in_bs, scale, nrel, blockIdx.x, eks);
+}
+template <int DT>
+__global__ __launch_bounds__(256) void att_presplit_rel_kernel(const float* __restrict__ q, const float* __restrict__ k,
+                                                               const float* __restrict__ v, uint4* __restrict__ kimg,
+                                                               uint4* __restrict__ vimg, const float* __restrict__ ek,
+                                                               float* __restrict__ relq, int H, int D, int T, int ld,
+                                                               long in_bs, float scale, int nrel, const int* lens,
+                                                               int* ovf_word, int* ovf_layer, int seq, int ntile) {
+  extern __shared__ float eks[];
+  const int x = __builtin_amdgcn_readfirstlane(blockIdx.x);
+  if (x < ntile) att_presplit_body<DT>(k, v, kimg, vimg, H, D, T, ld, in_bs, lens, ovf_word, ovf_layer, seq, x, ntile);
+  else rel_logits_body(q, ek, relq, H, D, T, ld, in_bs, scale, nrel, x - ntile, eks);
 }
 
 __global__ __launch_bounds__(256) void rel_values_kernel(const float* __restrict__ q, const float* __restrict__ k,
@@ -587,6 +613,112 @@
   }
 }
 
+__device__ __forceinline__ float att_add_rn(float a, float b) {
+#pragma clang fp contract(off)
+  return a + b;
+}
+
+__global__ __launch_bounds__(256) void attn_merge_rel_kernel(const float* __restrict__ opart, const float* __restrict__ q,
+                                                             const float* __restrict__ k, const float* __restrict__ relq,
+                                                             const float* __restrict__ ev, float* __restrict__ out, int H,
+                                                             int D, int DP, int T, int ld, long in_bs, long out_bs,
+                                                             float scale, int window, int nsplit, const int* lens) {
+  extern __shared__ float sm[];
+  const int nrel = 2 * window + 1;
+  const int KW = 64 + 2 * window;
+  const int dper = (D + 3) / 4;
+  float* ks = sm;
+  float* ps = ks + D * KW;
+  float* evs = ps + 64 * (nrel + 1);
+  const int tq = threadIdx.x & 63, part = __builtin_amdgcn_readfirstlane(threadIdx.x >> 6);
+  const int tb = blockIdx.x * 64, t = tb + tq;
+  const int hd = blockIdx.y >> 2, dq = blockIdx.y & 3, b = blockIdx.z;
+  const int d0 = dq * dper, d1 = min(D, d0 + dper);
+  const int len = lens ? lens[b] : T;
+  const long base = (long)b * in_bs + (long)hd * D * ld;
+  for (int idx = threadIdx.x; idx < D * KW; idx += 256) {
+    const int d = idx / KW, j = idx - d * KW;
+    const int key = tb - window + j;
+    ks[idx] = (key >= 0 && key < T) ? k[base + (long)d * ld + key] : 0.f;
+  }
+  for (int idx = threadIdx.x; idx < nrel * dper; idx += 256) {
+    const int r = idx / dper, dd = idx - r * dper;
+    evs[idx] = d0 + dd < d1 ? ev[r * D + d0 + dd] : 0.f;
+  }
+  const float* pb = opart + (((long)b * H + hd) * nsplit) * (DP + 2) * T;
+  const long ss = (long)(DP + 2) * T;
+  const int tc = min(t, T - 1);
+  float ms[8], w[8];
+  float m = -INFINITY, l = 0.f;
+#pragma unroll
+  for (int s = 0; s < 8; ++s) {
+    ms[s] = s < nsplit ? pb[s * ss + (long)DP * T + tc] : -INFINITY;
+    m = fmaxf(m, ms[s]);
+  }
+#pragma unroll
+  for (int s = 0; s < 8; ++s) {
+    w[s] = (ms[s] == -INFINITY) ? 0.f : expf(ms[s] - m);
+    if (s < nsplit) l += w[s] * pb[s * ss + (long)(DP + 1) * T + tc];
+  }
+  const float inv = 1.f / l;
+  __syncthreads();
+  if (t < T) {
+    const float* qb = q + base + t;
+    const float* rq = relq + (((long)b * H + hd) * T + t) * nrel;
+    const int nmine = part < nrel ? (nrel - part + 3) / 4 : 0;
+    float sacc[8];
+#pragma unroll
+    for (int i = 0; i < 8; ++i) sacc[i] = 0.f;
+    int d = 0;
+    for (; d + 8 <= D; d += 8) {
+      float qv[8];
+#pragma unroll
+      for (int u = 0; u < 8; ++u) qv[u] = qb[(long)(d + u) * ld] * scale;
+#pragma unroll
+      for (int i = 0; i < 8; ++i)
+        if (i < nmine) {
+          const float* kp = ks + d * KW + tq + part + 4 * i;
+#pragma unroll
+          for (int u = 0; u < 8; ++u) sacc[i] = fmaf(qv[u], kp[u * KW], sacc[i]);
+        }
+    }
+    for (; d < D; ++d) {
+      const float qv = qb[(long)d * ld] * scale;
+#pragma unroll
+      for (int i = 0; i < 8; ++i)
+        if (i < nmine) sacc[i] = fmaf(qv, ks[d * KW + tq + part + 4 * i], sacc[i]);
+    }
+#pragma unroll
+    for (int i = 0; i < 8; ++i)
+      if (i < nmine) {
+        const int r = part + 4 * i;
+        const int key = t + r - window;
+        float p = 0.f;
+        if (key >= 0 && key < len) {
+          const float s = sacc[i] + rq[r];
+          p = expf(s - m) / l;
+        }
+        ps[tq * (nrel + 1) + r] = p;
+      }
+  }
+  __syncthreads();
+  if (t >= T) return;
+  float* ob = out + (long)b * out_bs + (long)hd * D * ld;
+  for (int d = d0 + part; d < d1; d += 4) {
+    float acc = 0.f;
+#pragma unroll
+    for (int s = 0; s < 8; ++s)
+      if (s < nsplit) acc += w[s] * pb[s * ss + (long)d * T + t];
+    float o = t < len ? acc * inv : 0.f;
+    if (t < len) {
+      float ra = 0.f;
+      for (int r = 0; r < nrel; ++r) ra = fmaf(ps[tq * (nrel + 1) + r], evs[r * dper + d - d0], ra);
+      o = att_add_rn(o, ra);
+    }
+    ob[(long)d * ld + t] = o;
+  }
+}
+
 void launch_attention(const float* q, const float* k, const float* v, float* out, int B, int H, int D, int T,
                       int ld, long in_bs, long out_bs, float scale, const float* emb_rel_k, const float* emb_rel_v, int window,
                       const int* lens, float* scratch, float* split_scratch, hipStream_t stream, int* ovf, int* ovf_layer,
@@ -599,8 +731,6 @@
     relq = scratch;
     mb = relq + (size_t)B * H * T * nrel;
     lb = mb + (size_t)B * H * T;
-    hipLaunchKernelGGL(rel_logits_kernel, dim3(cdiv(T, 64), H, B), dim3(256), nrel * D * sizeof(float), stream,
-                       q, emb_rel_k, relq, H, D, T, ld, in_bs, scale, nrel);
   }
   const int DT = cdiv(D, 32);
   const long blocks = (long)cdiv(T, 128) * H;
@@ -620,22 +750,38 @@
   dim3 grid(cdiv(T, 128) * nsplit, H, B);
   static const int h3_env = getenv("RVCX_ATT_H3") ? atoi(getenv("RVCX_ATT_H3")) : 1;
   const int h3 = h3_env && !g_force_fp32 && allow_h3;
+  const bool fold = g_att_fold != 0 && h3 && nsplit > 1 && emb_rel_k && emb_rel_v;
+  if (emb_rel_k && !fold)
+    hipLaunchKernelGGL(rel_logits_kernel, dim3(cdiv(T, 64), H, B), dim3(256), nrel * D * sizeof(float), stream,
+                       q, emb_rel_k, relq, H, D, T, ld, in_bs, scale, nrel);
   if (h3) {
     RVCX_CHECK(split_scratch != nullptr, "attention: the split-fp16 kernel needs its scratch");
     const int ntile = cdiv(T, 32);
     uint4* kimg = reinterpret_cast<uint4*>(split_scratch + (size_t)B * H * 8 * 98 * T);
     uint4* vimg = kimg + (size_t)B * H * ntile * (DT * 256);
-    const dim3 pg(ntile, H, B);
+    const dim3 pg(ntile, H, B), pgr(ntile + cdiv(T, 64), H, B);
     if (DT == 1) {
-      hipLaunchKernelGGL(att_presplit_kernel<1>, pg, dim3(256), 0, stream, k, v, kimg, vimg, H, D, T, ld, in_bs, lens, ovf, ovf_layer, seq);
+      if (fold)
+        hipLaunchKernelGGL(att_presplit_rel_kernel<1>, pgr, dim3(256), nrel * D * sizeof(float), stream, q, k, v, kimg, vimg,
+                           emb_rel_k, relq, H, D, T, ld, in_bs, scale, nrel, lens, ovf, ovf_layer, seq, ntile);
+      else
+        hipLaunchKernelGGL(att_presplit_kernel<1>, pg, dim3(256), 0, stream, k, v, kimg, vimg, H, D, T, ld, in_bs, lens, ovf, ovf_layer, seq);
       hipLaunchKernelGGL(attn_h3_kernel<1>, grid, dim3(256), 0, stream, q, kimg, vimg, out, mo, lo, relq, H, D, T, ld, in_bs,
                          out_bs, scale, window, lens, nsplit, opart, ovf, ovf_layer, seq);
     } else if (DT == 2) {
-      hipLaunchKernelGGL(att_presplit_kernel<2>, pg, dim3(256), 0, stream, k, v, kimg, vimg, H, D, T, ld, in_bs, lens, ovf, ovf_layer, seq);
+      if (fold)
+        hipLaunchKernelGGL(att_presplit_rel_kernel<2>, pgr, dim3(256), nrel * D * sizeof(float), stream, q, k, v, kimg, vimg,
+                           emb_rel_k, relq, H, D, T, ld, in_bs, scale, nrel, lens, ovf, ovf_layer, seq, ntile);
+      else
+        hipLaunchKernelGGL(att_presplit_kernel<2>, pg, dim3(256), 0, stream, k, v, kimg, vimg, H, D, T, ld, in_bs, lens, ovf, ovf_layer, seq);
       hipLaunchKernelGGL(attn_h3_kernel<2>, grid, dim3(256), 0, stream, q, kimg, vimg, out, mo, lo, relq, H, D, T, ld, in_bs,
                          out_bs, scale, window, lens, nsplit, opart, ovf, ovf_layer, seq);
     } else {
-      hipLaunchKernelGGL(att_presplit_kernel<3>, pg, dim3(256), 0, stream, k, v, kimg, vimg, H, D, T, ld, in_bs, lens, ovf, ovf_layer, seq);
+      if (fold)
+        hipLaunchKernelGGL(att_presplit_rel_kernel<3>, pgr, dim3(256), nrel * D * sizeof(float), stream, q, k, v, kimg, vimg,
+                           emb_rel_k, relq, H, D, T, ld, in_bs, scale, nrel, lens, ovf, ovf_layer, seq, ntile);
+      else
+        hipLaunchKernelGGL(att_presplit_kernel<3>, pg, dim3(256), 0, stream, k, v, kimg, vimg, H, D, T, ld, in_bs, lens, ovf, ovf_layer, seq);
       hipLaunchKernelGGL(attn_h3_kernel<3>, grid, dim3(256), 0, stream, q, kimg, vimg, out, mo, lo, relq, H, D, T, ld, in_bs,
                          out_bs, scale, window, lens, nsplit, opart, ovf, ovf_layer, seq);
     }
@@ -649,6 +795,13 @@
   else
     hipLaunchKernelGGL(attn_kernel<3>, grid, dim3(256), 0, stream, q, k, v, out, mo, lo, relq, H, D, T, ld, in_bs,
                        out_bs, scale, window, lens, nsplit, opart);
+  if (fold) {
+    const size_t lds = ((size_t)D * (64 + 2 * window) + 64 * (nrel + 1) + (size_t)nrel * cdiv(D, 4)) * sizeof(float);
+    hipLaunchKernelGGL(attn_merge_rel_kernel, dim3(cdiv(T, 64), H * 4, B), dim3(256), lds, stream, opart, q, k, relq,
+                       emb_rel_v, out, H, D, 32 * DT, T, ld, in_bs, out_bs, scale, window, nsplit, lens);
+    RVCX_HIP(hipGetLastError());
+    return;
+  }
   if (nsplit > 1)
     hipLaunchKernelGGL(attn_merge_kernel, dim3(cdiv(T, 64), H * 4, B), dim3(256), 0, stream, opart, out, mb, lb, H, D,
                        32 * DT, T, ld, out_bs, nsplit, lens);
diff --git a/polgen-rvc_amd/csrc/ctx.h b/polgen-rvc_amd/csrc/ctx.h
--- a/polgen-rvc_amd/csrc/ctx.h
+++ b/polgen-rvc_amd/csrc/ctx.h
@@ -176,7 +176,7 @@
   hipEvent_t ev_io = nullptr;
   hipEvent_t ev_front[2] = {nullptr, nullptr};
   hipEvent_t ev_done[2] = {nullptr, nullptr};
-  hipEvent_t ev_src[2] = {nullptr, nullptr};
+  hipEvent_t ev_src[3] = {nullptr, nullptr, nullptr};
   Arena arena;
   size_t arena_budget = 0;
   Arena arena_f0;
diff --git a/polgen-rvc_amd/csrc/ops.h b/polgen-rvc_amd/csrc/ops.h
--- a/polgen-rvc_amd/csrc/ops.h
+++ b/polgen-rvc_amd/csrc/ops.h
@@ -3,6 +3,7 @@
 
 namespace rvcx {
 
+extern int g_att_fold;
 void launch_attention(const float* q, const float* k, const float* v, float* out, int B, int H, int D, int T,
                       int ld, long in_bs, long out_bs, float scale, const float* emb_rel_k, const float* emb_rel_v, int window,
                       const int* lens, float* scratch, float* split_scratch, hipStream_t stream,
diff --git a/polgen-rvc_amd/csrc/resblock.hip b/polgen-rvc_amd/csrc/resblock.hip
--- a/polgen-rvc_amd/csrc/resblock.hip
+++ b/polgen-rvc_amd/csrc/resblock.hip
@@ -1070,6 +1070,8 @@
   const H3Rsrc xr = h3_rsrc(a.x + (long)b * a.bs, C * a.cs * 4);
   const H3Rsrc w1r = h3_rsrc(a.w1, K * NCHUNK * 4 * C * 16);
   const H3Rsrc w2r = h3_rsrc(a.w2, K * NCHUNK * 4 * C * 16);
+  const bool sum_on = a.acc2_mode == ACC2_ADD || a.acc2_mode == ACC2_ADD_DIV;
+  const H3Rsrc y2r = h3_rsrc(sum_on ? a.y2 + (long)b * a.bs : a.x, sum_on ? C * a.cs * 4 : 0);
   const int xrow = a.cs * 4;
   constexpr int slab = 4 * C * 16;
 
@@ -1343,6 +1345,27 @@
         }
       }
     };
+    uint4 pq[WM][4];
+    auto request_sum = [&](int n) {
+      if (sum_on) {
+#pragma unroll
+        for (int m = 0; m < WM; ++m) {
+          const int col0 = wc * (WN * 32) + n * 32 + lc;
+          const int pos0 = n0 + col0;
+          const bool ok = col0 < BN_OUT && pos0 < a.T;
+#pragma unroll
+          for (int p = 0; p < 4; ++p) {
+            const int co = wr * (WM * 32) + m * 32 + lr + 8 * p;
+            pq[m][p] = h3_load4(y2r, ok ? (co * a.cs + pos0) * 4 : kH3Oob);
+          }
+        }
+      } else {
+#pragma unroll
+        for (int m = 0; m < WM; ++m)
+#pragma unroll
+          for (int p = 0; p < 4; ++p) pq[m][p] = make_uint4(0, 0, 0, 0);
+      }
+    };
     if (EARLY && NG == 1) request_res(0);
     for (int chunk = 0; chunk < NCHUNK; chunk += NCS) {
 #pragma unroll
@@ -1355,6 +1378,7 @@
         if (!last_stage) fetch_a(w2r, g + 1 == NG ? chunk + NCS : chunk, g + 1 == NG ? 0 : (g + 1) * KKT);
         else if (has_next) fetch_a(w1r, 0, 0);
         if (EARLY ? (NG > 1 && g == 0 && chunk + NCS >= NCHUNK) : last_stage) request_res(0);
+        if (last_stage) request_sum(0);
         if (NG > 1 && g == NG - 1) compute(Last{}, Y1 + chunk * 4 * N1P, N1P, 4 * N1P, g * KKT, 1);
         else compute(Full{}, Y1 + chunk * 4 * N1P, N1P, 4 * N1P, g * KKT, 1);
       }
@@ -1368,7 +1392,13 @@
 #pragma unroll
       for (int n = 1; n < WN; ++n) request_res(n);
 #pragma unroll
-      for (int n = 0; n < WN; ++n)
+      for (int n = 0; n < WN; ++n) {
+        float4 pv[WM][4];
+#pragma unroll
+        for (int m = 0; m < WM; ++m)
+#pragma unroll
+          for (int p = 0; p < 4; ++p) pv[m][p] = __builtin_bit_cast(float4, pq[m][p]);
+        if (n + 1 < WN) request_sum(n + 1);
 #pragma unroll
         for (int m = 0; m < WM; ++m) {
 #pragma unroll
@@ -1377,15 +1407,9 @@
           const int col0 = wc * (WN * 32) + n * 32 + lc;
           const int pos0 = n0 + col0;
           const bool ok = col0 < BN_OUT && pos0 < a.T;
-          float4 v[4], pv[4];
-#pragma unroll
-          for (int p = 0; p < 4; ++p) {
-            const int co = wr * (WM * 32) + m * 32 + lr + 8 * p;
-            const long off = (long)b * a.bs + (long)co * a.cs + pos0;
-            v[p] = *reinterpret_cast<const float4*>(stg + (lr + 8 * p) * P + lc);
-            pv[p] = (ok && a.acc2_mode != ACC2_NONE && a.acc2_mode != ACC2_SET) ? *reinterpret_cast<const float4*>(a.y2 + off)
-                                                                                : make_float4(0.f, 0.f, 0.f, 0.f);
-          }
+          float4 v[4];
+#pragma unroll
+          for (int p = 0; p < 4; ++p) v[p] = *reinterpret_cast<const float4*>(stg + (lr + 8 * p) * P + lc);
           __builtin_amdgcn_wave_barrier();
           if (ok) {
 #pragma unroll
@@ -1399,7 +1423,7 @@
               for (int q = 0; q < 4; ++q) o[q] = pos0 + q < len ? o[q] : 0.f;
               if (a.y) *reinterpret_cast<float4*>(a.y + off) = make_float4(o[0], o[1], o[2], o[3]);
               if (a.acc2_mode != ACC2_NONE) {
-                const float pp[4] = {pv[p].x, pv[p].y, pv[p].z, pv[p].w};
+                const float pp[4] = {pv[m][p].x, pv[m][p].y, pv[m][p].z, pv[m][p].w};
 #pragma unroll
                 for (int q = 0; q < 4; ++q) {
                   if (a.acc2_mode == ACC2_ADD) o[q] = pp[q] + o[q];
@@ -1410,6 +1434,7 @@
             }
           }
         }
+      }
     }
     stamp(5);
   }
diff --git a/polgen-rvc_amd/csrc/synth.hip b/polgen-rvc_amd/csrc/synth.hip
--- a/polgen-rvc_amd/csrc/synth.hip
+++ b/polgen-rvc_amd/csrc/synth.hip
@@ -254,12 +254,33 @@
                   S.noise.k <= fuse_max_k;
     (void)probe;
   }
+  float* g = A.alloc<float>((size_t)B * gin);
+  float* gc4 = A.alloc<float>((size_t)4 * B * 6 * hid);
+  float* gcond = A.alloc<float>((size_t)B * cf.up_initial_channel);
+  bool equal_lens = true;
+  if (io.lens_host)
+    for (int b = 1; b < B; ++b) equal_lens &= io.lens_host[b] == io.lens_host[0];
+  static const int dec_batch_env = getenv("RVCX_DEC_BATCH") ? std::max(1, atoi(getenv("RVCX_DEC_BATCH"))) : 8;
+  const int dec_batch = equal_lens ? dec_batch_env : 1;
   {
     hipStream_t sn = c.serial ? s : c.aux[0];
     if (sn != s) {
       RVCX_HIP(hipEventRecord(c.ev_src[0], s));
       RVCX_HIP(hipStreamWaitEvent(sn, c.ev_src[0], 0));
     }
+    for (int b = 0; b < B; ++b)
+      RVCX_HIP(hipMemcpyAsync(g + (size_t)b * gin, m.emb_g + (size_t)sidv[b] * gin, gin * sizeof(float),
+                              hipMemcpyDeviceToDevice, sn));
+    for (int f = 3; f >= 0; --f) {
+      ConvArgs a = conv1d_args(m.flows[f].cond, g, gc4 + (size_t)f * B * 6 * hid, B, 1, 1);
+      c.conv_on(a, sn);
+    }
+    for (int b0 = 0; b0 < B; b0 += dec_batch) {
+      const int db = std::min(dec_batch, B - b0);
+      ConvArgs a = conv1d_args(m.cond, g + (size_t)b0 * gin, gcond + (size_t)b0 * cf.up_initial_channel, db, 1, 1);
+      c.conv_on(a, sn);
+    }
+    if (sn != s) RVCX_HIP(hipEventRecord(c.ev_src[2], sn));
     double* sc = A.alloc<double>((size_t)B * Tk * 2);
     launch_sine_source(pitchf, io.src_noise, har, B, Tk, m.upp, (float)cf.sr, m.lin_wb, lens, sc, sn);
     long tt = Tk;
@@ -343,10 +364,7 @@
     launch_copy_strided(z + head, z2, B * inter, Tk, T, Tk, s);
     std::swap(z, z2);
   }
-  float* g = A.alloc<float>((size_t)B * gin);
-  for (int b = 0; b < B; ++b)
-    RVCX_HIP(hipMemcpyAsync(g + (size_t)b * gin, m.emb_g + (size_t)sidv[b] * gin, gin * sizeof(float),
-                            hipMemcpyDeviceToDevice, s));
+  if (!c.serial) RVCX_HIP(hipStreamWaitEvent(s, c.ev_src[2], 0));
   {
     float* h = att;
     float* xin = qkv;
@@ -355,16 +373,14 @@
     RVCX_CHECK(filt >= 2 * hid, "buffer reuse assumes filter_channels >= 2*hidden");
     float* wout = A.alloc<float>((size_t)B * hid * T);
     float* mbuf = A.alloc<float>((size_t)B * half * T);
-    float* gc = A.alloc<float>((size_t)B * 6 * hid);
     for (int f = 3; f >= 0; --f) {
       const auto& F = m.flows[f];
+      const float* gc = gc4 + (size_t)f * B * 6 * hid;
       launch_flip_channels(z, z2, B, inter, Tk, s);
       std::swap(z, z2);
       ConvArgs a = conv1d_args(F.pre, z, h, B, Tk, Tk);
       a.x_bs = (long)inter * Tk;
       a.lens_out = lens;
-      c.conv(a);
-      a = conv1d_args(F.cond, g, gc, B, 1, 1);
       c.conv(a);
       for (int i = 0; i < 3; ++i) {
         a = conv1d_args(F.in_l[i], h, xin, B, Tk, Tk, 1, 1, (F.in_l[i].k - 1) / 2);
@@ -389,11 +405,6 @@
   if (io.ev_decoder) RVCX_HIP(hipEventRecord(io.ev_decoder, s));
 
   if (!c.serial) RVCX_HIP(hipStreamWaitEvent(s, c.ev_src[1], 0));
-  static const int dec_batch_env = getenv("RVCX_DEC_BATCH") ? std::max(1, atoi(getenv("RVCX_DEC_BATCH"))) : 8;
-  bool equal_lens = true;
-  if (io.lens_host)
-    for (int b = 1; b < B; ++b) equal_lens &= io.lens_host[b] == io.lens_host[0];
-  const int dec_batch = equal_lens ? dec_batch_env : 1;
   const int C0 = cf.up_initial_channel;
   const size_t dec_mark = A.mark();
   for (int b0 = 0; b0 < B; b0 += dec_batch) {
@@ -411,10 +422,7 @@
       a.x_cs = Tk;
       a.lens_in = (lens && !own) ? lens + b0 : nullptr;
       c.conv(a);
-      float* gcond = A.alloc<float>((size_t)db * C0);
-      a = conv1d_args(m.cond, g + (size_t)b0 * gin, gcond, db, 1, 1);
-      c.conv(a);
-      launch_add_channel_bias(cur, gcond, db, C0, Td, s);
+      launch_add_channel_bias(cur, gcond + (size_t)b0 * C0, db, C0, Td, s);
     }
     long Tin = Td, Tin_c = Tk, off = skip;
     for (size_t i = 0; i < m.stages.size(); ++i) {
```

Result: no change. 1250 (median of 2 runs) (+0.1%).
